# edlanglois/relearn

Hardware: AMD Instinct MI355X
Metric: env-steps/sec (whole node), 64k-env CartPole TRPO (higher is better)
Workload: dtype f32; 1 GPU; CartPole(VisibleStepLimit 500) MLP-TRPO, 65536 envs total, T=128, policy 5-128-2, critic 5-128-1, CG 10, <=15 backtracks, 80 Adam critic steps per period; n_envs_total=65536, n_envs_per_gpu=65536, horizon=128, hidden=128, critic_steps=80, update_chains=policy and critic chains side by side on two streams, pipeline=none, parallelism=env-sharded x1 + no collective (one rank)

## Files before the change

### include/relearn_hip.h

```cpp
#ifndef RELEARN_HIP_H
#define RELEARN_HIP_H

#include <stddef.h>
#include <stdint.h>

#ifdef __cplusplus
extern "C" {
#endif

#define RL_ABI_VERSION 6

typedef enum {
  RL_OK = 0,
  RL_ERR_INVALID_ARGUMENT = 1,
  RL_ERR_HIP = 2,
  RL_ERR_NO_DEVICE = 3,
  RL_ERR_BUILD_AGENT = 4,
  RL_ERR_BUILD_ENV = 5,
  RL_ERR_BUFFER_FULL = 6,
  RL_ERR_PACKING = 7,
  RL_ERR_COMM = 8,
  RL_ERR_OPT_NAN = 9,
  RL_ERR_UNSUPPORTED = 10
} rl_status;
// ... 82 lines not shown
int32_t rl_env_reset(rl_env *env);
int32_t rl_env_observe(rl_env *env, float *obs_out);
int32_t rl_env_step(rl_env *env, const uint8_t *actions, float *reward_out, uint8_t *flag_out, float *obs_out,
                    float *term_obs_out);
int32_t rl_env_upload_actions(rl_env *env, const uint8_t *actions);
int32_t rl_env_step_resident(rl_env *env);
int32_t rl_env_get_state(rl_env *env, double *state4, int32_t *nv_pos, uint64_t *steps_remaining,
                         uint64_t *reset_count);
int32_t rl_env_set_state(rl_env *env, const double *state4, const int32_t *nv_pos, const uint64_t *steps_remaining,
                         const uint64_t *reset_count);

int32_t rl_debug_stream_words(rl_engine *engine, uint64_t seed, uint64_t stream, uint64_t first_word, uint32_t n_words,
                              uint32_t *words_out);
int32_t rl_debug_device_memory(uint64_t *live_bytes, uint64_t *live_allocations);

int32_t rl_mlp_create(rl_engine *engine, uint32_t in_dim, uint32_t hidden, uint32_t out_dim, rl_mlp **out);
typedef enum {
  RL_ACT_IDENTITY = 0,
  RL_ACT_RELU = 1,
  RL_ACT_SIGMOID = 2,
  RL_ACT_TANH = 3
} rl_activation;
int32_t rl_mlp_create_layers(rl_engine *engine, uint32_t in_dim, const uint32_t *hidden_sizes, uint32_t n_hidden,
                             uint32_t out_dim, int32_t activation, int32_t output_activation, rl_mlp **out);
int32_t rl_mlp_create_config(rl_engine *engine, uint32_t in_dim, const uint32_t *hidden_sizes, uint32_t n_hidden,
                             uint32_t out_dim, int32_t activation, int32_t output_activation, int32_t bias, rl_mlp **out);
int32_t rl_mlp_destroy(rl_mlp *mlp);
int32_t rl_mlp_num_params(const rl_mlp *mlp, uint64_t *n);
int32_t rl_mlp_init(rl_mlp *mlp, uint64_t seed);
typedef enum { RL_INIT_ZEROS = 0, RL_INIT_CONSTANT = 1, RL_INIT_UNIFORM = 2, RL_INIT_NORMAL = 3, RL_INIT_ORTHOGONAL = 4 } rl_init_kind;
typedef enum { RL_SCALE_CONSTANT = 0, RL_SCALE_FAN_IN = 1, RL_SCALE_FAN_OUT = 2, RL_SCALE_FAN_AVG = 3 } rl_variance_scale;
typedef struct {
  int32_t kind;
  int32_t scale;
  double value;
} rl_initializer;
int32_t rl_mlp_init_with(rl_mlp *mlp, uint64_t seed, const rl_initializer *kernel_init, const rl_initializer *bias_init);
int32_t rl_rnn_mlp_init_with(rl_mlp *module, uint64_t seed, const rl_initializer *input_weights_init,
                             const rl_initializer *hidden_weights_init, const rl_initializer *bias_init,
                             const rl_initializer *mlp_kernel_init, const rl_initializer *mlp_bias_init);
int32_t rl_params_get(rl_mlp *mlp, float *host, uint64_t n);
int32_t rl_params_set(rl_mlp *mlp, const float *host, uint64_t n);
int32_t rl_mlp_forward(rl_mlp *mlp, const float *rows, uint64_t n_rows, float *out);

int32_t rl_gru_mlp_create(rl_engine *engine, uint32_t in_dim, uint32_t gru_hidden, uint32_t mlp_hidden,
                          uint32_t out_dim, rl_mlp **out);
int32_t rl_lstm_mlp_create(rl_engine *engine, uint32_t in_dim, uint32_t lstm_hidden, uint32_t mlp_hidden,
                           uint32_t out_dim, rl_mlp **out);
enum { RL_CELL_GRU = 0, RL_CELL_LSTM = 1 };
int32_t rl_rnn_mlp_create(rl_engine *engine, int32_t cell, uint32_t in_dim, uint32_t hidden_size, uint32_t num_layers,
                          uint32_t mlp_hidden, uint32_t out_dim, rl_mlp **out);
int32_t rl_rnn_mlp_create_config(rl_engine *engine, int32_t cell, uint32_t in_dim, uint32_t hidden_size,
                                 uint32_t num_layers, int32_t bias, uint32_t mlp_hidden, uint32_t out_dim, rl_mlp **out);

typedef enum {
  RL_TRAJ_OBS = 0,
  RL_TRAJ_ACTION = 1,
  RL_TRAJ_REWARD = 2,
  RL_TRAJ_FLAG = 3,
  RL_TRAJ_TERM_OBS = 4,
  RL_TRAJ_VALUES = 5,
  RL_TRAJ_ADVANTAGES = 6,
  RL_TRAJ_RETURNS = 7,
  RL_TRAJ_TARGETS = 8
} rl_traj_field;

int32_t rl_traj_create(rl_engine *engine, uint64_t n_lanes, uint64_t horizon, uint32_t obs_dim, rl_traj **out);
int32_t rl_traj_destroy(rl_traj *traj);
int32_t rl_traj_field_bytes(const rl_traj *traj, int32_t field, uint64_t *bytes);
int32_t rl_traj_read(rl_traj *traj, int32_t field, void *host, uint64_t bytes);
int32_t rl_traj_write(rl_traj *traj, int32_t field, const void *host, uint64_t bytes);

int32_t rl_rollout(rl_env *env, const rl_mlp *policy, rl_traj *traj);

int32_t rl_gae(rl_traj *traj, const rl_mlp *critic, float gamma, float lambda);
int32_t rl_seq_forward(rl_mlp *module, rl_traj *traj, float *out, float *succ_out);

typedef struct {
  uint64_t iterations;
  uint64_t max_backtracks;
  double backtrack_ratio;
  double hpv_reg_coeff;
  double max_policy_step_kl;
  int32_t accept_violation;
} rl_trpo_config;
int32_t rl_trpo_config_default(rl_trpo_config *cfg);

typedef struct {
  double entropy, step_size, loss_initial, loss_final, constraint_val_final, step_scale;
  int64_t num_backtracks;
  int32_t status;
  int32_t cg_iterations;
} rl_trpo_stats;

int32_t rl_trpo_update(rl_mlp *policy, rl_traj *traj, const rl_trpo_config *cfg, rl_trpo_stats *stats);
int32_t rl_policy_gradient(rl_mlp *policy, rl_traj *traj, float *grad_out, float *loss_out, float *entropy_out);
int32_t rl_policy_fvp(rl_mlp *policy, rl_traj *traj, const float *v, float reg, float *out);
int32_t rl_policy_loss_kl(rl_mlp *policy, rl_traj *traj, const float *params0, float *loss_out, float *kl_out);

typedef struct {
  double learning_rate, beta1, beta2, weight_decay;
  double eps;
} rl_adam_config;
int32_t rl_adam_config_default(rl_adam_config *cfg);
int32_t rl_adam_create(rl_mlp *module, const rl_adam_config *cfg, rl_adam **out);
int32_t rl_adam_destroy(rl_adam *opt);
int32_t rl_adam_step_host(rl_adam *opt, const float *grad);

enum { RL_OPTIMIZER_ADAM = 0, RL_OPTIMIZER_ADAMW = 1, RL_OPTIMIZER_SGD = 2, RL_OPTIMIZER_RMSPROP = 3 };
typedef struct {
  int32_t kind;
  int32_t nesterov;
  int32_t centered;
  int32_t reserved;
  double learning_rate, weight_decay;
  double beta1, beta2;
  double eps;
  double momentum, dampening;
  double alpha;
} rl_optimizer_config;
int32_t rl_optimizer_config_default(int32_t kind, rl_optimizer_config *cfg);
int32_t rl_optimizer_create(rl_mlp *module, const rl_optimizer_config *cfg, rl_adam **out);
int32_t rl_optimizer_step_host(rl_adam *opt, const float *grad);
int32_t rl_optimizer_state_read(rl_adam *opt, int32_t slot, float *host, uint64_t n, uint64_t *step_out);

typedef struct {
  double loss_first, loss_last;
  uint64_t steps;
} rl_critic_stats;
int32_t rl_critic_update(rl_mlp *critic, rl_adam *opt, rl_traj *traj, uint64_t opt_steps, rl_critic_stats *stats,
                         float *losses_out);
int32_t rl_critic_gradient(rl_mlp *critic, rl_traj *traj, float *grad_out, float *loss_out);

enum { RL_VALUE_TARGET_REWARD_TO_GO = 0, RL_VALUE_TARGET_ONE_STEP_TD = 1 };
typedef struct {
  uint64_t opt_steps_per_update;
  int32_t target;
  float discount_factor;
} rl_values_opt_config;
int32_t rl_values_opt_config_default(rl_values_opt_config *cfg);
int32_t rl_values_opt_update(rl_mlp *critic, rl_adam *opt, rl_traj *traj, const rl_values_opt_config *cfg,
                             rl_critic_stats *stats, float *losses_out );

int32_t rl_actor_critic_update(rl_mlp *policy, rl_mlp *critic, rl_adam *critic_opt, rl_traj *traj,
                               const rl_trpo_config *policy_cfg, const rl_values_opt_config *critic_cfg,
                               rl_trpo_stats *policy_stats, rl_critic_stats *critic_stats ,
                               float *critic_losses_out );
int32_t rl_actor_critic_update_begin(rl_mlp *policy, rl_mlp *critic, rl_adam *critic_opt, rl_traj *traj,
                                     const rl_trpo_config *policy_cfg, const rl_values_opt_config *critic_cfg,
                                     rl_trpo_stats *policy_stats);
int32_t rl_actor_critic_update_finish(rl_traj *traj, rl_critic_stats *critic_stats ,
                                      float *critic_losses_out );
int32_t rl_engine_set_serial_update(rl_engine *engine, int32_t serial);

typedef struct {
  uint64_t opt_steps_per_update;
  double clip_distance;
} rl_ppo_config;
int32_t rl_ppo_config_default(rl_ppo_config *cfg);
typedef struct {
  double entropy;
  double loss_first, loss_last;
  uint64_t steps;
} rl_policy_opt_stats;
int32_t rl_ppo_update(rl_mlp *policy, rl_adam *opt, rl_traj *traj, const rl_ppo_config *cfg,
                      rl_policy_opt_stats *stats, float *losses_out );
int32_t rl_reinforce_update(rl_mlp *policy, rl_adam *opt, rl_traj *traj, rl_policy_opt_stats *stats);
int32_t rl_reward_to_go(rl_traj *traj, float gamma);

enum { RL_DQN_TARGET_REWARD_TO_GO = 0, RL_DQN_TARGET_ONE_STEP_TD = 1 };
enum { RL_SCHEDULE_CONSTANT = 0, RL_SCHEDULE_LINEAR_ANNEALED = 1 };
enum { RL_COLLECT_CONSTANT = 0, RL_COLLECT_FIRST_REST = 1 };
typedef struct {
  int32_t target;
  int32_t exploration_kind;
  double exploration_start, exploration_end;
  uint64_t exploration_period;
  uint64_t minibatch_steps;
  uint64_t opt_steps_per_update;
  uint64_t buffer_capacity;
  uint64_t episode_capacity;
  int32_t update_kind;
  uint64_t update_first, update_rest;
  float discount_factor;
  uint32_t agent_key[8];
} rl_dqn_config;
int32_t rl_dqn_config_default(rl_dqn_config *cfg);
int32_t rl_dqn_create(rl_env *env, rl_mlp *qnet, rl_adam *opt, const rl_dqn_config *cfg, rl_dqn **out);
int32_t rl_dqn_destroy(rl_dqn *dqn);
int32_t rl_dqn_exploration_rate(const rl_dqn *dqn, int32_t training, double *rate_out);
int32_t rl_dqn_min_update_size(const rl_dqn *dqn, uint64_t *min_steps_out, uint64_t *slack_steps_out);
typedef struct {
  double exploration_rate;
  uint64_t steps;
  uint64_t episodes_ended;
} rl_dqn_collect_stats;
int32_t rl_dqn_collect(rl_dqn *dqn, uint64_t horizon, rl_dqn_collect_stats *stats );
typedef struct {
  double loss_first, loss_last;
  uint64_t opt_steps;
  uint64_t global_steps;
  uint64_t last_minibatch_steps, last_minibatch_episodes;
} rl_dqn_update_stats;
int32_t rl_dqn_update(rl_dqn *dqn, rl_dqn_update_stats *stats, float *losses_out );

enum { RL_REPLAY_HEAD = 0, RL_REPLAY_COUNT = 1, RL_REPLAY_EP_HEAD = 2, RL_REPLAY_EP_COUNT = 3, RL_REPLAY_TOTAL = 4,
       RL_REPLAY_EP_END = 5 , RL_REPLAY_OBS = 6 , RL_REPLAY_NEXT_OBS = 7,
       RL_REPLAY_ACTION = 8 , RL_REPLAY_REWARD = 9 , RL_REPLAY_FLAG = 10 ,
       RL_REPLAY_ACTOR_POS = 11 , RL_REPLAY_LAST_FLAGS = 12  };
int32_t rl_dqn_replay_field_bytes(const rl_dqn *dqn, int32_t field, uint64_t *bytes);
int32_t rl_dqn_replay_read(rl_dqn *dqn, int32_t field, void *host, uint64_t bytes);
int32_t rl_dqn_minibatch_sample(rl_dqn *dqn, int32_t sequential, uint64_t *n_episodes_out, uint64_t *n_steps_out);
enum { RL_MB_EP_LANE = 0, RL_MB_EP_START = 1, RL_MB_EP_LEN = 2, RL_MB_EP_OFFSET = 3 ,
       RL_MB_OBS = 4 , RL_MB_ACTION = 5 , RL_MB_TARGET = 6  };
int32_t rl_dqn_minibatch_read(rl_dqn *dqn, int32_t field, void *host, uint64_t bytes);
int32_t rl_dqn_minibatch_gradient(rl_dqn *dqn, float *grad_out, float *loss_out);
int32_t rl_dqn_agent_rng_pos(rl_dqn *dqn, uint64_t *pos_out);

typedef struct {
  double mean;
  double squared_residual_sum;
  uint64_t count;
} rl_mean_variance;
typedef struct {
  rl_mean_variance step_reward;
  rl_mean_variance episode_reward;
  rl_mean_variance episode_length;
} rl_steps_summary;
int32_t rl_summary_create(rl_engine *engine, uint64_t n_lanes, rl_summary **out);
int32_t rl_summary_destroy(rl_summary *s);
int32_t rl_summary_push(rl_summary *s, const rl_traj *traj);
int32_t rl_summary_push_dqn(rl_summary *s, const rl_dqn *dqn);
int32_t rl_summary_read(rl_summary *s, rl_steps_summary *out);
int32_t rl_summary_clear(rl_summary *s, int32_t forget_episodes_in_progress);
int32_t rl_steps_summary_merge(const rl_steps_summary *a, const rl_steps_summary *b, rl_steps_summary *out);

enum { RL_ACTOR_POLICY = 0, RL_ACTOR_DQN = 1 };
int32_t rl_actor_to_cbor(rl_env *env, rl_mlp *module, int32_t actor_kind, double exploration_rate, uint8_t *buf,
                         uint64_t cap, uint64_t *len_out);
int32_t rl_module_from_cbor(rl_mlp *module, const uint8_t *buf, uint64_t len);

typedef enum {
  RL_KIND_UINT8 = 0, RL_KIND_INT8 = 1, RL_KIND_INT16 = 2, RL_KIND_INT = 3, RL_KIND_INT64 = 4, RL_KIND_HALF = 5,
  RL_KIND_FLOAT = 6, RL_KIND_DOUBLE = 7, RL_KIND_COMPLEX_HALF = 8, RL_KIND_COMPLEX_FLOAT = 9,
  RL_KIND_COMPLEX_DOUBLE = 10, RL_KIND_BOOL = 11, RL_KIND_QINT8 = 12, RL_KIND_QUINT8 = 13, RL_KIND_QINT32 = 14,
  RL_KIND_BFLOAT16 = 15
} rl_tensor_kind;
int32_t rl_tensor_def_to_cbor(int32_t kind, const int64_t *shape, uint32_t rank, int32_t requires_grad,
                              const void *data, uint64_t data_bytes, uint8_t *buf, uint64_t cap, uint64_t *len_out);
int32_t rl_tensor_def_from_cbor(const uint8_t *buf, uint64_t len, int32_t *kind_out, int64_t *shape_out,
                                uint32_t shape_cap, uint32_t *rank_out, int32_t *requires_grad_out, void *data_out,
                                uint64_t data_cap, uint64_t *data_bytes_out);
int32_t rl_indexed_type_space_to_cbor(uint8_t *buf, uint64_t cap, uint64_t *len_out);

int32_t rl_chain_tabular_q_train(uint64_t seed, uint64_t n_threads, uint64_t n_periods, uint64_t min_worker_steps,
                                 double exploration_rate, double *q_values_out, uint64_t *counts_out,
                                 uint64_t *total_steps_out);
int32_t rl_chain_tabular_q_eval(const double *q_values, uint64_t seed, uint64_t n_steps, uint8_t *actions_out,
                                double *total_reward_out);

#ifdef __cplusplus
}
#endif
#endif
```

### relearn_amd/__init__.py

```python
import atexit
import ctypes as C
import math
import os
import subprocess
import sys
import weakref

import numpy as np

_HERE = os.path.dirname(os.path.abspath(__file__))
LIB_PATH = os.environ.get("RELEARN_LIB", os.path.join(_HERE, "librelearn_hip.so"))
CSRC = os.path.join(_HERE, "csrc")

OK = 0
ERR_INVALID_ARGUMENT, ERR_HIP, ERR_NO_DEVICE, ERR_BUILD_AGENT, ERR_BUILD_ENV = 1, 2, 3, 4, 5
ERR_BUFFER_FULL, ERR_PACKING, ERR_COMM, ERR_OPT_NAN, ERR_UNSUPPORTED = 6, 7, 8, 9, 10
SUCC_CONTINUE, SUCC_TERMINATE, SUCC_INTERRUPT = 0, 1, 2
OPT_OK, OPT_LOSS_NOT_IMPROVING, OPT_CONSTRAINT_VIOLATED, OPT_NAN_LOSS, OPT_NAN_CONSTRAINT = range(5)
ENV_CARTPOLE, ENV_CHAIN, ENV_MEMORY, ENV_BANDIT, ENV_META_BANDIT = 0, 1, 2, 3, 4
BANDITS_UNIFORM_BERNOULLI, BANDITS_ONE_HOT, BANDITS_ROUND_ROBIN = 0, 1, 2
BANDIT_DISTRIBUTIONS = {"uniform_bernoulli": BANDITS_UNIFORM_BERNOULLI, "one_hot": BANDITS_ONE_HOT,
                        "round_robin": BANDITS_ROUND_ROBIN}
LIMIT_NONE, LIMIT_LATENT, LIMIT_VISIBLE = 0, 1, 2
(TRAJ_OBS, TRAJ_ACTION, TRAJ_REWARD, TRAJ_FLAG, TRAJ_TERM_OBS, TRAJ_VALUES, TRAJ_ADVANTAGES,
 TRAJ_RETURNS, TRAJ_TARGETS) = range(9)
VALUE_TARGET_REWARD_TO_GO, VALUE_TARGET_ONE_STEP_TD = 0, 1
OPTIMIZER_ADAM, OPTIMIZER_ADAMW, OPTIMIZER_SGD, OPTIMIZER_RMSPROP = 0, 1, 2, 3
KERNEL_CLASSES = ["env_step", "rollout", "values", "gae", "policy_pass", "backward", "reduce", "small",
                  "critic_fwd", "allreduce", "critic_fused", "policy_fused", "policy_fvp"]

ABI_SYMBOLS = [
    "rl_abi_version", "rl_debug_stream_words", "rl_debug_device_memory", "rl_device_count", "rl_engine_create", "rl_engine_destroy", "rl_engine_sync",
    "rl_last_error", "rl_engine_info", "rl_engine_set_kernel_variant", "rl_timer_begin", "rl_timer_end", "rl_profile_enable", "rl_profile_read",
    "rl_comm_available", "rl_comm_library_paths", "rl_comm_unique_id", "rl_comm_init", "rl_comm_destroy", "rl_comm_init_host",
    "rl_comm_ipc_handle", "rl_comm_init_ipc", "rl_comm_selftest",
    "rl_cartpole_params_default", "rl_env_create", "rl_env_create_bandit", "rl_meta_bandit_config_default", "rl_env_create_meta_bandit", "rl_env_destroy", "rl_env_dims", "rl_env_reset",
    "rl_env_observe", "rl_env_step", "rl_env_upload_actions", "rl_env_step_resident", "rl_env_get_state",
    "rl_env_set_state",
    "rl_mlp_create", "rl_mlp_create_layers", "rl_mlp_create_config", "rl_mlp_destroy", "rl_mlp_num_params", "rl_mlp_init", "rl_mlp_init_with", "rl_params_get", "rl_params_set",
    "rl_mlp_forward", "rl_gru_mlp_create", "rl_lstm_mlp_create", "rl_rnn_mlp_create", "rl_rnn_mlp_create_config", "rl_rnn_mlp_init_with", "rl_seq_forward",
    "rl_traj_create", "rl_traj_destroy", "rl_traj_field_bytes", "rl_traj_read", "rl_traj_write",
    "rl_rollout", "rl_gae",
    "rl_trpo_config_default", "rl_trpo_update", "rl_policy_gradient", "rl_policy_fvp", "rl_policy_loss_kl",
    "rl_adam_config_default", "rl_adam_create", "rl_adam_destroy", "rl_adam_step_host",
    "rl_optimizer_config_default", "rl_optimizer_create", "rl_optimizer_step_host", "rl_optimizer_state_read",
    "rl_critic_update", "rl_critic_gradient", "rl_values_opt_config_default", "rl_values_opt_update",
    "rl_actor_critic_update", "rl_actor_critic_update_begin", "rl_actor_critic_update_finish", "rl_engine_set_serial_update",
    "rl_ppo_config_default", "rl_ppo_update", "rl_reinforce_update", "rl_reward_to_go",
    "rl_actor_to_cbor", "rl_module_from_cbor", "rl_tensor_def_to_cbor", "rl_tensor_def_from_cbor",
    "rl_indexed_type_space_to_cbor",
    "rl_dqn_config_default", "rl_dqn_create", "rl_dqn_destroy", "rl_dqn_exploration_rate",
    "rl_dqn_min_update_size", "rl_dqn_collect", "rl_dqn_update", "rl_dqn_replay_field_bytes", "rl_dqn_replay_read",
    "rl_dqn_minibatch_sample", "rl_dqn_minibatch_read", "rl_dqn_minibatch_gradient", "rl_dqn_agent_rng_pos",
    "rl_chain_tabular_q_train", "rl_chain_tabular_q_eval",
    "rl_summary_create", "rl_summary_destroy", "rl_summary_push", "rl_summary_push_dqn", "rl_summary_read",
    "rl_summary_clear", "rl_steps_summary_merge",
]


HOST_ALLREDUCE_FN = C.CFUNCTYPE(C.c_int32, C.c_void_p, C.POINTER(C.c_float), C.c_uint64)


class RelearnError(RuntimeError):
    def __init__(self, code, message):
        super().__init__("rl status %d: %s" % (code, message))
        self.code = code


class CartPoleParams(C.Structure):
    _fields_ = [(n, C.c_double) for n in (
        "gravity", "mass_cart", "mass_pole", "length_half_pole", "friction_cart", "friction_pole", "time_step",
        "action_force", "max_pos", "max_angle", "discount_factor")]


class EnvConfig(C.Structure):
    _fields_ = [("kind", C.c_int32), ("limit_kind", C.c_int32), ("max_steps", C.c_uint64), ("n_lanes", C.c_uint64),
                ("lane_offset", C.c_uint64), ("seed_env", C.c_uint64), ("seed_actor", C.c_uint64),
                ("cartpole", CartPoleParams), ("chain_size", C.c_uint64), ("memory_num_actions", C.c_uint64),
                ("memory_history_len", C.c_uint64), ("bandit_values", C.c_double * 2)]


class MetaBanditConfig(C.Structure):
    _fields_ = [("n_arms", C.c_uint32), ("distribution", C.c_int32), ("episodes_per_trial", C.c_uint64)]


class TrpoConfig(C.Structure):
    _fields_ = [("iterations", C.c_uint64), ("max_backtracks", C.c_uint64), ("backtrack_ratio", C.c_double),
                ("hpv_reg_coeff", C.c_double), ("max_policy_step_kl", C.c_double), ("accept_violation", C.c_int32)]


class TrpoStats(C.Structure):
    _fields_ = [("entropy", C.c_double), ("step_size", C.c_double), ("loss_initial", C.c_double),
                ("loss_final", C.c_double), ("constraint_val_final", C.c_double), ("step_scale", C.c_double),
                ("num_backtracks", C.c_int64), ("status", C.c_int32), ("cg_iterations", C.c_int32)]

    def as_dict(self):
        return {k: getattr(self, k) for k, _ in self._fields_}


class AdamConfig(C.Structure):
    _fields_ = [("learning_rate", C.c_double), ("beta1", C.c_double), ("beta2", C.c_double),
                ("weight_decay", C.c_double), ("eps", C.c_double)]


class OptimizerConfig(C.Structure):
    _fields_ = [("kind", C.c_int32), ("nesterov", C.c_int32), ("centered", C.c_int32), ("reserved", C.c_int32),
                ("learning_rate", C.c_double), ("weight_decay", C.c_double), ("beta1", C.c_double),
                ("beta2", C.c_double), ("eps", C.c_double), ("momentum", C.c_double), ("dampening", C.c_double),
                ("alpha", C.c_double)]


class CriticStats(C.Structure):
    _fields_ = [("loss_first", C.c_double), ("loss_last", C.c_double), ("steps", C.c_uint64)]


def build(force=False, check=False):
    if force or check or not os.path.exists(LIB_PATH):
        before = os.path.getmtime(LIB_PATH) if os.path.exists(LIB_PATH) else None
        subprocess.check_call(["make", "-C", CSRC, "-s", "-j4"] + (["-B"] if force else []))
        _write_build_record(before)
    return LIB_PATH


BUILD_RECORD = os.path.join(_HERE, "build_record.json")


def _write_build_record(mtime_before):
    import hashlib
    import json
    import time
    try:
        after = os.path.getmtime(LIB_PATH)
        try:
            hipcc = subprocess.run(["/opt/rocm/bin/hipcc", "--version"], capture_output=True, timeout=30).stdout.decode().splitlines()[0]
        except Exception:
            hipcc = None
        rec = {"mode": "linked a new library" if mtime_before is None or after > mtime_before else
                       "make: library newer than every source (nothing compiled)",
               "lib_sha16": hashlib.sha256(open(LIB_PATH, "rb").read()).hexdigest()[:16],
               "lib_mtime": time.strftime("%Y-%m-%dT%H:%M:%SZ", time.gmtime(after)),
               "checked_at": time.strftime("%Y-%m-%dT%H:%M:%SZ", time.gmtime()), "hipcc": hipcc,
               "arch": "gfx950"}
        json.dump(rec, open(BUILD_RECORD, "w"), indent=1)
    except Exception:
        pass


_lib = None


def lib():
    global _lib
    if _lib is None:
        if not os.path.exists(LIB_PATH):
            raise ImportError("librelearn_hip.so is not built: run `python -c 'import __graft_entry__ as g; "
                              "g.build()'` (there is no CPU fallback)")
        L = C.CDLL(LIB_PATH)
        L.rl_last_error.restype = C.c_char_p
        L.rl_last_error.argtypes = [C.c_void_p]
        _lib = L
    return _lib


def debug_device_memory():
    nbytes, count = C.c_uint64(), C.c_uint64()
    _check(lib().rl_debug_device_memory(C.byref(nbytes), C.byref(count)))
    return nbytes.value, count.value


def _check(code, eng=None):
    if code != OK:
        msg = lib().rl_last_error(eng)
        raise RelearnError(code, msg.decode() if msg else "")


def _ptr(a, dtype):
    a = np.ascontiguousarray(a, dtype=dtype)
    return a, a.ctypes.data_as(C.c_void_p)


_live = weakref.WeakSet()


def _register(obj):
    _live.add(obj)


@atexit.register
def _close_all():
    objs = list(_live)
    order = {"StepsSummary": -1, "Dqn": -1, "Adam": 0, "Optimizer": 0, "Trajectory": 1, "CartPoleEnv": 2, "ChainEnv": 2, "MetaBanditEnv": 2, "Mlp": 3, "GruMlp": 3,
             "Engine": 4}
    for o in sorted(objs, key=lambda o: order.get(type(o).__name__, 2)):
        o.close()


class _Handle:
    def __del__(self):
        if sys.is_finalizing():
            return
        try:
            self.close()
        except Exception:
            pass


class Engine(_Handle):
    def __init__(self, device=0):
        self.h = C.c_void_p()
        _check(lib().rl_engine_create(C.c_int32(device), C.byref(self.h)))
        _register(self)

    def close(self):
        if self.h:
            lib().rl_engine_destroy(self.h)
            self.h = C.c_void_p()

    def sync(self):
        _check(lib().rl_engine_sync(self.h), self.h)

    def info(self):
        name = C.create_string_buffer(256)
        arch = C.create_string_buffer(256)
        cus = C.c_int32()
        _check(lib().rl_engine_info(self.h, name, C.c_size_t(256), arch, C.c_size_t(256), C.byref(cus)), self.h)
        return name.value.decode(), arch.value.decode(), cus.value

    def stream_words(self, seed, stream, first_word, n_words):
        out = np.zeros(n_words, dtype=np.uint32)
        _check(lib().rl_debug_stream_words(self.h, C.c_uint64(seed), C.c_uint64(stream), C.c_uint64(first_word),
                                           C.c_uint32(n_words), out.ctypes.data_as(C.c_void_p)), self.h)
        return out

    def set_kernel_variant(self, variant):
        _check(lib().rl_engine_set_kernel_variant(self.h, C.c_int32(variant)), self.h)

    def set_serial_update(self, serial):
        _check(lib().rl_engine_set_serial_update(self.h, C.c_int32(1 if serial else 0)), self.h)

    def timer_begin(self):
        _check(lib().rl_timer_begin(self.h), self.h)

    def timer_end(self):
        ms = C.c_float()
        _check(lib().rl_timer_end(self.h, C.byref(ms)), self.h)
        return ms.value

    def profile_enable(self, on=True):
        _check(lib().rl_profile_enable(self.h, C.c_int32(1 if on else 0)), self.h)

    def profile_read(self, reset=True):
        ms = (C.c_double * len(KERNEL_CLASSES))()
        cnt = (C.c_uint64 * len(KERNEL_CLASSES))()
        _check(lib().rl_profile_read(self.h, ms, cnt, C.c_int32(1 if reset else 0)), self.h)
        return {k: (ms[i], cnt[i]) for i, k in enumerate(KERNEL_CLASSES)}

    def comm_init(self, rank, n_ranks, unique_id):
        buf = (C.c_uint8 * 128).from_buffer_copy(bytes(unique_id))
        _check(lib().rl_comm_init(self.h, C.c_int32(rank), C.c_int32(n_ranks), buf), self.h)

    def comm_ipc_handle(self, n_ranks):
        buf = (C.c_uint8 * 64)()
        _check(lib().rl_comm_ipc_handle(self.h, C.c_int32(n_ranks), buf), self.h)
        return bytes(buf)

    def comm_init_ipc(self, rank, n_ranks, handles):
        blob = b"".join(bytes(h) for h in handles)
        assert len(blob) == 64 * n_ranks
        buf = (C.c_uint8 * len(blob)).from_buffer_copy(blob)
        _check(lib().rl_comm_init_ipc(self.h, C.c_int32(rank), C.c_int32(n_ranks), buf), self.h)

    def comm_selftest(self):
        _check(lib().rl_comm_selftest(self.h), self.h)

    def comm_destroy(self):
        _check(lib().rl_comm_destroy(self.h), self.h)
        self._host_allreduce = None

    def comm_init_host(self, rank, n_ranks, allreduce):
        def thunk(_ctx, buf, count):
            try:
                allreduce(np.ctypeslib.as_array(buf, shape=(count,)))
                return 0
            except Exception:
                import traceback
                traceback.print_exc()
                return 1
        self._host_allreduce = HOST_ALLREDUCE_FN(thunk)
        _check(lib().rl_comm_init_host(self.h, C.c_int32(rank), C.c_int32(n_ranks), self._host_allreduce, None),
               self.h)


def comm_available():
    return lib().rl_comm_available() == OK


def comm_library_paths():
    a, b = C.create_string_buffer(1024), C.create_string_buffer(1024)
    _check(lib().rl_comm_library_paths(a, C.c_size_t(1024), b, C.c_size_t(1024)))
    return a.value.decode(), b.value.decode()


def comm_unique_id():
    buf = (C.c_uint8 * 128)()
    _check(lib().rl_comm_unique_id(buf))
    return bytes(buf)


def cartpole_params_default():
    p = CartPoleParams()
    _check(lib().rl_cartpole_params_default(C.byref(p)))
    return p


class CartPoleEnv(_Handle):

    def __init__(self, engine, n_lanes, max_steps=500, limit=LIMIT_VISIBLE, lane_offset=0, seed_env=0,
                 seed_actor=1, params=None):
        self.eng = engine
        cfg = EnvConfig()
        cfg.kind = ENV_CARTPOLE
        cfg.limit_kind = limit
        cfg.max_steps = max_steps
        cfg.n_lanes = n_lanes
        cfg.lane_offset = lane_offset
        cfg.seed_env = seed_env
        cfg.seed_actor = seed_actor
        cfg.cartpole = params if params is not None else cartpole_params_default()
        self.cfg = cfg
        self.h = C.c_void_p()
        _check(lib().rl_env_create(engine.h, C.byref(cfg), C.byref(self.h)), engine.h)
        _register(self)
        self.n = n_lanes
        d, a = C.c_uint32(), C.c_uint32()
        _check(lib().rl_env_dims(self.h, C.byref(d), C.byref(a)), engine.h)
        self.D, self.A = d.value, a.value

    def close(self):
        if self.h:
            lib().rl_env_destroy(self.h)
            self.h = C.c_void_p()

    def reset(self):
        _check(lib().rl_env_reset(self.h), self.eng.h)

    def observe(self):
        obs = np.zeros((self.D, self.n), dtype=np.float32)
        _check(lib().rl_env_observe(self.h, obs.ctypes.data_as(C.c_void_p)), self.eng.h)
        return obs

    def step(self, actions):
        a, ap = _ptr(actions, np.uint8)
        assert a.shape == (self.n,)
        reward = np.zeros(self.n, dtype=np.float32)
        flag = np.zeros(self.n, dtype=np.uint8)
        obs = np.zeros((self.D, self.n), dtype=np.float32)
        term = np.zeros((self.D, self.n), dtype=np.float32)
        _check(lib().rl_env_step(self.h, ap, reward.ctypes.data_as(C.c_void_p), flag.ctypes.data_as(C.c_void_p),
                                 obs.ctypes.data_as(C.c_void_p), term.ctypes.data_as(C.c_void_p)), self.eng.h)
        return reward, flag, obs, term

    def upload_actions(self, actions):
        a, ap = _ptr(actions, np.uint8)
        _check(lib().rl_env_upload_actions(self.h, ap), self.eng.h)

    def step_resident(self):
        _check(lib().rl_env_step_resident(self.h), self.eng.h)

    def get_state(self):
        st = np.zeros((4, self.n), dtype=np.float64)
        nv = np.zeros(self.n, dtype=np.int32)
        rem = np.zeros(self.n, dtype=np.uint64)
        rc = np.zeros(self.n, dtype=np.uint64)
        _check(lib().rl_env_get_state(self.h, st.ctypes.data_as(C.c_void_p), nv.ctypes.data_as(C.c_void_p),
                                      rem.ctypes.data_as(C.c_void_p), rc.ctypes.data_as(C.c_void_p)), self.eng.h)
        return st, nv, rem, rc

    def set_state(self, st, nv, rem, rc):
        st, sp = _ptr(st, np.float64)
        nv, np_ = _ptr(nv, np.int32)
        rem, rp = _ptr(rem, np.uint64)
        rc, cp = _ptr(rc, np.uint64)
        _check(lib().rl_env_set_state(self.h, sp, np_, rp, cp), self.eng.h)


class ChainEnv(_Handle):

    def __init__(self, engine, n_lanes, max_steps=100, limit=LIMIT_LATENT, lane_offset=0, seed_env=0, seed_actor=1):
        self.eng = engine
        cfg = EnvConfig()
        cfg.kind = ENV_CHAIN
        cfg.limit_kind = limit
# ... 746 lines not shown
```

### relearn_amd/csrc/abi.hip

```cpp
#include <dlfcn.h>

#include <atomic>
#include <condition_variable>
#include <map>
#include <mutex>

#include "abi_internal.hpp"
#include "env_lanes.hpp"

thread_local std::string g_last_error_no_engine;

static std::atomic<uint64_t> g_device_bytes{0}, g_device_allocations{0};

void *rl_device_alloc(uint64_t bytes) {
  void *p = nullptr;
  RL_HIP_CHECK(hipMalloc(&p, bytes));
  g_device_bytes += bytes;
  g_device_allocations += 1;
  return p;
}

void rl_device_free(void *p, uint64_t bytes) {
  (void)hipFree(p);
  g_device_bytes -= bytes;
// ... 170 lines not shown
    RL_HIP_CHECK(hipStreamSynchronize(e->stream));
    return;
  }
  if (!e->comm) {
    if (e->n_ranks > 1) throw RlError(RL_ERR_COMM, "engine has n_ranks > 1 but no collective (rl_comm_init failed?)");
    return;
  }
  ProfScope ps(e, RL_K_ALLREDUCE);
  void *comm = e->chan == 1 && e->comm_aux ? e->comm_aux : e->comm;
  rccl_check(g_rccl.AllReduce(d_buf, d_buf, count, 7, 0, comm, e->stream), "ncclAllReduce");
}

void comm_agree(rl_engine *e) {
  const bool mine = std::getenv("RELEARN_SERIAL_UPDATE") != nullptr;
  if (!e->has_collective()) {
    e->agreed_serial_env = mine;
    return;
  }
  float h[2] = {mine ? 1.0f : 0.0f, 1.0f};
  {
    DevMem tmp;
    float *d = tmp.alloc<float>(2);
    h2d(e, d, h, sizeof(h));
    rl_allreduce_sum_f32(e, d, 2);
    d2h(e, h, d, sizeof(h));
    ipc_check(e);
  }
  if (h[1] != (float)e->n_ranks)
    throw RlError(RL_ERR_COMM, "the collective's first all-reduce counted " + std::to_string((int)h[1]) + " of " +
                                   std::to_string(e->n_ranks) + " ranks");
  e->agreed_serial_env = h[0] != 0.0f;
}

extern "C" {

int32_t rl_abi_version(void) { return RL_ABI_VERSION; }

int32_t rl_device_count(int32_t *count) {
  return guarded(nullptr, [&] {
    RL_REQUIRE(count, "count is NULL");
    int n = 0;
    if (hipGetDeviceCount(&n) != hipSuccess) n = 0;
    *count = n;
  });
}

int32_t rl_engine_create(int32_t device_ordinal, rl_engine **out) {
  return guarded(nullptr, [&] {
    RL_REQUIRE(out, "out is NULL");
    *out = nullptr;
    int n = 0;
    if (hipGetDeviceCount(&n) != hipSuccess || n <= 0)
      throw RlError(RL_ERR_NO_DEVICE, "no HIP device visible: this engine has no CPU fallback");
    RL_REQUIRE(device_ordinal >= 0 && device_ordinal < n, "device ordinal out of range");
    std::unique_ptr<rl_engine> e(new rl_engine());
    e->device = device_ordinal;
    RL_HIP_CHECK(hipSetDevice(device_ordinal));
    RL_HIP_CHECK(hipGetDeviceProperties(&e->prop, device_ordinal));
    if (std::strncmp(e->prop.gcnArchName, "gfx950", 6) != 0)
      throw RlError(RL_ERR_NO_DEVICE,
                    std::string("device is ") + e->prop.gcnArchName + ", this library is built for gfx950 only");
    RL_HIP_CHECK(hipStreamCreateWithFlags(&e->main_stream, hipStreamNonBlocking));
    RL_HIP_CHECK(hipStreamCreateWithFlags(&e->aux_stream, hipStreamNonBlocking));
    e->stream = e->main_stream;
    RL_HIP_CHECK(hipEventCreateWithFlags(&e->ev_fork, hipEventDisableTiming));
    RL_HIP_CHECK(hipEventCreateWithFlags(&e->ev_join, hipEventDisableTiming));
    RL_HIP_CHECK(hipEventCreate(&e->ev_begin));
    RL_HIP_CHECK(hipEventCreate(&e->ev_end));
    e->pinned_bytes = 1 << 16;
    RL_HIP_CHECK(hipHostMalloc(&e->pinned, e->pinned_bytes, hipHostMallocDefault));
    *out = e.release();
  });
}

static void engine_teardown(rl_engine *e);

int32_t rl_engine_destroy(rl_engine *e) {
  if (!e) return RL_OK;
  if (e->live_handles > 0) {
    e->zombie = true;
    return RL_OK;
  }
  engine_teardown(e);
  return RL_OK;
}

void engine_release_child(rl_engine *e) {
  e->live_handles -= 1;
  if (e->zombie && e->live_handles <= 0) engine_teardown(e);
}

static void engine_teardown(rl_engine *e) {
  (void)hipSetDevice(e->device);
  (void)hipStreamSynchronize(e->main_stream);
  (void)hipStreamSynchronize(e->aux_stream);
  if (e->comm_aux && g_rccl.CommDestroy) g_rccl.CommDestroy(e->comm_aux);
  if (e->comm && g_rccl.CommDestroy) g_rccl.CommDestroy(e->comm);
  ipc_teardown(e);
  prof_drain(e);
  for (auto ev : e->prof_event_pool) (void)hipEventDestroy(ev);
  if (e->pinned) (void)hipHostFree(e->pinned);
  (void)hipEventDestroy(e->ev_begin);
  (void)hipEventDestroy(e->ev_end);
  (void)hipEventDestroy(e->ev_fork);
  (void)hipEventDestroy(e->ev_join);
  (void)hipStreamDestroy(e->aux_stream);
  (void)hipStreamDestroy(e->main_stream);
  delete e;
}

int32_t rl_engine_sync(rl_engine *e) {
  return guarded(e, [&] {
    RL_REQUIRE(e, "engine is NULL");
    sync(e);
    RL_HIP_CHECK(hipSetDevice(e->device));
    RL_HIP_CHECK(hipDeviceSynchronize());
    ipc_check(e);
  });
}

const char *rl_last_error(const rl_engine *e) { return e ? e->last_error.c_str() : g_last_error_no_engine.c_str(); }

int32_t rl_engine_info(const rl_engine *e, char *name_out, size_t name_cap, char *arch_out, size_t arch_cap,
                       int32_t *compute_units) {
  return guarded(const_cast<rl_engine *>(e), [&] {
    RL_REQUIRE(e, "engine is NULL");
    if (name_out && name_cap) std::snprintf(name_out, name_cap, "%s", e->prop.name[0] ? e->prop.name : e->prop.gcnArchName);
    if (arch_out && arch_cap) std::snprintf(arch_out, arch_cap, "%s", e->prop.gcnArchName);
    if (compute_units) *compute_units = e->prop.multiProcessorCount;
  });
}

int32_t rl_timer_begin(rl_engine *e) {
  return guarded(e, [&] {
    RL_REQUIRE(e, "engine is NULL");
    RL_HIP_CHECK(hipEventRecord(e->ev_begin, e->stream));
  });
}

int32_t rl_timer_end(rl_engine *e, float *elapsed_ms) {
  return guarded(e, [&] {
    RL_REQUIRE(e && elapsed_ms, "NULL argument");
    RL_HIP_CHECK(hipEventRecord(e->ev_end, e->stream));
    RL_HIP_CHECK(hipEventSynchronize(e->ev_end));
    RL_HIP_CHECK(hipEventElapsedTime(elapsed_ms, e->ev_begin, e->ev_end));
  });
}

int32_t rl_engine_set_kernel_variant(rl_engine *e, int32_t variant) {
  return guarded(e, [&] {
    RL_REQUIRE(e, "engine is NULL");
    RL_REQUIRE(variant == 0 || variant == 1, "kernel variant must be 0 (best) or 1 (v1 reference kernels)");
    e->kernel_variant = variant;
  });
}

int32_t rl_engine_set_serial_update(rl_engine *e, int32_t serial) {
  return guarded(e, [&] {
    RL_REQUIRE(e, "engine is NULL");
    e->serial_update = serial != 0;
  });
}

int32_t rl_profile_enable(rl_engine *e, int32_t on) {
  return guarded(e, [&] {
    RL_REQUIRE(e, "engine is NULL");
    sync(e);
    prof_drain(e);
    e->profiling = on != 0;
  });
}

int32_t rl_profile_read(rl_engine *e, double *total_ms_out, uint64_t *launches_out, int32_t reset) {
  return guarded(e, [&] {
    RL_REQUIRE(e, "engine is NULL");
    sync(e);
    prof_drain(e);
    for (int i = 0; i < RL_K_CLASS_COUNT; ++i) {
      if (total_ms_out) total_ms_out[i] = e->prof_ms[i];
      if (launches_out) launches_out[i] = e->prof_launches[i];
      if (reset) {
        e->prof_ms[i] = 0.0;
        e->prof_launches[i] = 0;
      }
    }
  });
}

int32_t rl_comm_available(void) {
  return guarded(nullptr, [&] {
    if (std::getenv("RELEARN_LOOPBACK_COMM")) return;
    rccl_load();
  });
}

int32_t rl_comm_library_paths(char *rccl_out, size_t rccl_cap, char *hip_out, size_t hip_cap) {
  return guarded(nullptr, [&] {
    Dl_info info;
    if (rccl_out && rccl_cap) {
      rccl_out[0] = 0;
      if (g_rccl.AllReduce && dladdr((void *)g_rccl.AllReduce, &info) != 0 && info.dli_fname)
        std::snprintf(rccl_out, rccl_cap, "%s", info.dli_fname);
    }
    if (hip_out && hip_cap) {
      hip_out[0] = 0;
      if (dladdr((void *)&hipGetDeviceCount, &info) != 0 && info.dli_fname)
        std::snprintf(hip_out, hip_cap, "%s", info.dli_fname);
    }
  });
}

int32_t rl_comm_unique_id(uint8_t id_out[128]) {
  return guarded(nullptr, [&] {
    RL_REQUIRE(id_out, "id_out is NULL");
    if (std::getenv("RELEARN_LOOPBACK_COMM")) {
      static std::atomic<uint64_t> counter{0};
      std::memset(id_out, 0, 128);
      uint64_t v = ++counter;
      std::memcpy(id_out, &v, sizeof(v));
      return;
    }
    rccl_load();
    rccl_check(g_rccl.GetUniqueId(id_out), "ncclGetUniqueId");
  });
}

int32_t rl_comm_init(rl_engine *e, int32_t rank, int32_t n_ranks, const uint8_t unique_id[128]) {
  return guarded(e, [&] {
    RL_REQUIRE(e && unique_id, "NULL argument");
    RL_REQUIRE(n_ranks >= 1 && rank >= 0 && rank < n_ranks, "bad rank / n_ranks");
    RL_REQUIRE(!e->has_collective(), "communicator already initialised");
    if (std::getenv("RELEARN_LOOPBACK_COMM")) {
      RL_REQUIRE(!e->loopback, "communicator already initialised");
      std::lock_guard<std::mutex> lk(g_loopback_mu);
      std::string key((const char *)unique_id, 128);
      auto &grp = g_loopback_groups[key];
      if (!grp) {
        grp = std::make_shared<LoopbackGroup>();
        grp->n_ranks = n_ranks;
        grp->bufs.assign(n_ranks, nullptr);
        RL_HIP_CHECK(hipSetDevice(e->device));
        RL_HIP_CHECK(hipMalloc((void **)&grp->d_bufs, n_ranks * sizeof(float *)));
        if (const char *tw = std::getenv("RELEARN_LOOPBACK_TEST_WEIGHT")) {
          int r = -1;
          float w = 1.0f;
          if (std::sscanf(tw, "%d:%f", &r, &w) == 2 && r >= 0 && r < n_ranks) grp->bad_rank = r, grp->bad_weight = w;
        }
      }
      RL_REQUIRE(grp->n_ranks == n_ranks, "loopback group: inconsistent n_ranks");
      grp->joined += 1;
      e->loopback = grp.get();
      e->rank = rank;
      e->n_ranks = n_ranks;
      e->agreed_serial_env = std::getenv("RELEARN_SERIAL_UPDATE") != nullptr;
      return;
    }
    if (n_ranks == 1 && !std::getenv("RELEARN_FORCE_RCCL")) return;
    rccl_load();
    RL_HIP_CHECK(hipSetDevice(e->device));
    UniqueId id;
    std::memcpy(id.bytes, unique_id, 128);
    comm_init_rank_t init = (comm_init_rank_t)(void *)g_rccl.CommInitRank;
    void *comm = nullptr;
    rccl_check(init(&comm, n_ranks, id, rank), "ncclCommInitRank");
    e->comm = comm;
    e->rank = rank;
    e->n_ranks = n_ranks;
    try {
      const bool want_aux = std::getenv("RELEARN_NO_AUX_COMM") == nullptr;
      UniqueId id2;
      std::memset(id2.bytes, 0, sizeof(id2.bytes));
      bool id_ok = false;
      if (rank == 0 && want_aux) id_ok = g_rccl.GetUniqueId(id2.bytes) == 0;
      float h_id[130];
      for (int i = 0; i < 128; ++i) h_id[i] = rank == 0 && id_ok ? (float)(unsigned char)id2.bytes[i] : 0.0f;
      h_id[128] = rank == 0 && !id_ok ? 1.0f : 0.0f;
      h_id[129] = want_aux ? 0.0f : 1.0f;
      DevMem tmp;
      float *d_id = tmp.alloc<float>(130);
      void *comm2 = nullptr;
      try {
        h2d(e, d_id, h_id, sizeof(h_id));
        rccl_check(g_rccl.AllReduce(d_id, d_id, 130, 7, 0, e->comm, e->stream), "ncclAllReduce (second unique id)");
        d2h(e, h_id, d_id, sizeof(h_id));
        const bool attempt = h_id[128] == 0.0f && h_id[129] == 0.0f;
        float outcome = 0.0f;
        if (attempt) {
          for (int i = 0; i < 128; ++i) id2.bytes[i] = (char)(unsigned char)h_id[i];
          if (init(&comm2, n_ranks, id2, rank) == 0 && comm2 != nullptr) outcome = 1.0f;
          else comm2 = nullptr;
        }
        h2d(e, d_id, &outcome, sizeof(outcome));
        rccl_check(g_rccl.AllReduce(d_id, d_id, 1, 7, 0, e->comm, e->stream), "ncclAllReduce (second communicator: outcome)");
        d2h(e, &outcome, d_id, sizeof(outcome));
        if (outcome == (float)n_ranks) {
          e->comm_aux = comm2;
          comm2 = nullptr;
        } else {
          if (rank == 0)
            std::fprintf(stderr, "relearn_hip: no second communicator (%s): update chains will run one after the other "
                                 "on every rank\n",
                         !attempt ? (h_id[129] != 0.0f ? "RELEARN_NO_AUX_COMM on some rank" : "rank 0 could not make an id")
                                  : "ncclCommInitRank failed on some rank");
        }
      } catch (...) {
        if (comm2) g_rccl.CommDestroy(comm2);
// ... 1101 lines not shown
```

### relearn_amd/csrc/abi_internal.hpp

```cpp
#pragma once
#include <cmath>
#include <cstdlib>
#include <cstring>
#include <memory>
#include <string>
#include <vector>

#include "../../include/rl_chacha.h"
#include "../../include/rl_detmath.h"
#include "engine.hpp"
#include "host/cbor.hpp"
#include "kernels.hpp"

extern thread_local std::string g_last_error_no_engine;

static inline void engine_settle(rl_engine *e) {
  if (e->pending.active && !e->pending.joined) {
    RL_HIP_CHECK(hipStreamWaitEvent(e->main_stream, e->ev_join, 0));
    e->pending.joined = true;
  }
}

template <typename F>
static inline int32_t guarded(rl_engine *eng, F &&f, bool settle = true) {
  try {
    if (eng != nullptr) eng->call_epoch += 1;
    if (eng != nullptr && settle) engine_settle(eng);
    f();
    if (eng != nullptr) {
      const hipError_t le = hipGetLastError();
      if (le != hipSuccess) throw RlError(RL_ERR_HIP, std::string("kernel launch failed: ") + hipGetErrorString(le));
    }
    return RL_OK;
  } catch (const RlError &e) {
    if (eng != nullptr) eng->error_epoch += 1;
    (eng ? eng->last_error : g_last_error_no_engine) = e.what();
    return e.code;
  } catch (const std::exception &e) {
    if (eng != nullptr) eng->error_epoch += 1;
    (eng ? eng->last_error : g_last_error_no_engine) = e.what();
    return RL_ERR_INVALID_ARGUMENT;
  } catch (...) {
    if (eng != nullptr) eng->error_epoch += 1;
    (eng ? eng->last_error : g_last_error_no_engine) = "unknown error";
    return RL_ERR_INVALID_ARGUMENT;
  }
}

static inline uint64_t b_total(const rl_traj *t) { return t->B * (uint64_t)t->eng->n_ranks; }

static inline void sync(rl_engine *e) { RL_HIP_CHECK(hipStreamSynchronize(e->stream)); }

static inline void h2d(rl_engine *e, void *d, const void *h, size_t bytes) {
  RL_HIP_CHECK(hipMemcpyAsync(d, h, bytes, hipMemcpyHostToDevice, e->stream));
  sync(e);
}

static inline void d2h(rl_engine *e, void *h, const void *d, size_t bytes) {
  RL_HIP_CHECK(hipMemcpyAsync(h, d, bytes, hipMemcpyDeviceToHost, e->stream));
  sync(e);
}

constexpr uint32_t RL_GUARD_BOTH = (1u << RL_GUARD_POLICY) | (1u << RL_GUARD_CRITIC);
static inline void range_check(rl_traj *t, uint32_t chains = RL_GUARD_BOTH) {
  if (chains & (1u << RL_GUARD_POLICY)) t->guard_next_policy = true;
  if (chains & (1u << RL_GUARD_CRITIC)) t->guard_next_critic = true;
  if (t->h_range_err == nullptr) return;
  volatile uint32_t *w = t->h_range_err;
  uint32_t seen = 0u;
  for (int c = 0; c < 2; ++c)
    if ((chains & (1u << c)) != 0u && w[c] != 0u) seen |= 1u << c;
  if (seen == 0u) return;
  for (int c = 0; c < 2; ++c)
    if (seen & (1u << c)) {
      w[c] = 0u;
      RL_HIP_CHECK(hipMemsetAsync(t->d.range + RL_RANGE_WORDS + c, 0, sizeof(uint32_t), t->eng->stream));
    }
  sync(t->eng);
  throw RlError(RL_ERR_UNSUPPORTED,
                std::string("numeric range of the fused update kernels exceeded in the ") +
                    (seen == RL_GUARD_BOTH ? "policy and critic chains" : (seen & 1u) ? "policy chain" : "critic chain") +
                    " (|pre-activation| bound 2^31 or a non-zero pre-activation below 2^-46 possible, or a non-finite "
                    "observation): the result of this call is not valid and the update was not applied; use "
                    "rl_engine_set_kernel_variant(engine, 1) for these magnitudes (include/relearn_hip.h)");
}
static inline void range_discard(rl_traj *t) {
  try {
    range_check(t);
  } catch (const RlError &) {
  }
}

enum PassKind { RUN_INIT = PASS_INIT, RUN_EVAL = PASS_EVAL, RUN_JVP = PASS_JVP, RUN_DQN = PASS_DQN, RUN_PPO = PASS_PPO,
                RUN_CRITIC, RUN_KINDS };
struct SlabRows {
  uint32_t A, B;
};
struct PassRequest {
  PassRequest(PassKind k) : kind(k) {}
  PassKind kind;
  const float *tangent = nullptr;
  const int32_t *skip = nullptr;
  float clip_lo = 0.0f, clip_hi = 0.0f;
  bool forward_only = false;
  bool reduce = true;
  uint64_t B_total = 0;
};
SlabRows run_pass(const rl_mlp *mod, rl_traj *traj, const PassRequest &req);

extern "C" {
void engine_release_child(rl_engine *e);
void traj_plan(rl_traj *t, uint64_t B);
rl_traj *traj_alloc(rl_engine *e, uint64_t n_lanes, uint64_t horizon, uint32_t obs_dim, bool resizable);
void seq_ensure(rl_traj *t, const rl_mlp *mod, bool training);
void traj_ensure_pvec(rl_traj *t, uint64_t P);
rl_mlp *seq_exec(const rl_mlp *m);
}

struct SeqScope {
  rl_traj *t;
  uint32_t logical_D;
  rl_mlp *x;
  SeqScope(rl_traj *traj, const rl_mlp *m) : t(traj), logical_D(traj->d.D), x(nullptr) {
    RL_REQUIRE(m->in_dim == traj->d.D, "module input width does not match the trajectory");
    x = seq_exec(m);
    if (!m->lane_kernels()) t->d.D = 5;
  }
  ~SeqScope() { t->d.D = logical_D; }
  SeqScope(const SeqScope &) = delete;
  SeqScope &operator=(const SeqScope &) = delete;
};
```

### relearn_amd/csrc/abi_update.hip

```cpp
#include "abi_internal.hpp"

enum FusedLauncher { FUSED_NONE, FUSED_POLICY ,
                     FUSED_CRITIC  };
struct PassRow {
  bool backward, sums;
  FusedLauncher fused;
};
static const PassRow PASS_TABLE[RUN_KINDS] = {
     {true, true, FUSED_POLICY},
     {false, true, FUSED_POLICY},
     {true, false, FUSED_POLICY},
     {true, true, FUSED_NONE},
     {true, true, FUSED_POLICY},
     {true, true, FUSED_CRITIC},
};
static_assert(RUN_INIT == 0 && RUN_EVAL == 1 && RUN_JVP == 2 && RUN_DQN == 3 && RUN_PPO == 4 && RUN_CRITIC == 5 &&
                  RUN_KINDS == 6,
              "PASS_TABLE rows are in the order of PassKind");

static void seq_gradient_to_flat_order(const rl_mlp *mod, rl_traj *traj) {
  if (mod->exec == nullptr) return;
  launch_seq_unpad(mod, traj->vec, mod->x_tmp);
  RL_HIP_CHECK(hipMemcpyAsync(traj->vec, mod->x_tmp, mod->P * sizeof(float), hipMemcpyDeviceToDevice, traj->eng->stream));
}

static float *seq_record(rl_traj *traj, const rl_mlp *mod) {
  return mod->lane_kernels() ? traj->seq.stack.rec : traj->seq.act;
}

SlabRows run_pass(const rl_mlp *mod, rl_traj *traj, const PassRequest &req) {
  const PassRow &row = PASS_TABLE[req.kind];
  const bool critic = req.kind == RUN_CRITIC;
  const uint32_t P = (uint32_t)mod->P;
  const uint64_t Bt = req.B_total ? req.B_total : b_total(traj);
  bool grad = row.backward;
  auto allreduce = [&] {
    rl_allreduce_sum_f32(traj->eng, traj->vec + (grad ? 0 : P), (grad ? P : 0) + (row.sums ? 4 : 0));
  };
  if (rl_module_is_recurrent(mod->kind)) {
    RL_REQUIRE(req.reduce, "a recurrent pass reduces its own sums");
    grad = row.backward && !req.forward_only;
    SeqScope sc(traj, mod);
    seq_ensure(traj, sc.x, true);
    if (req.kind == RUN_JVP) {
      const float *tangent = req.tangent;
      if (mod->exec != nullptr) {
        launch_seq_pad(mod, mod->x_tan, req.tangent);
        tangent = mod->x_tan;
      }
      launch_gru_tangent(traj, sc.x, tangent, Bt, req.skip);
    } else {
      launch_gru_seq_forward(traj, sc.x, traj->seq.out, nullptr, grad ? seq_record(traj, sc.x) : nullptr, req.skip);
      if (critic) launch_seq_critic_dvalues(traj, Bt);
      else launch_seq_policy_dlogits(traj, req.kind, Bt, req.clip_lo, req.clip_hi, req.skip);
    }
    if (grad) {
      launch_gru_backward(traj, sc.x, req.skip);
      seq_gradient_to_flat_order(mod, traj);
    }
    if (row.sums) launch_reduce(traj, P, false, true, 0, traj->nbB);
    allreduce();
    return SlabRows{0, traj->nbB};
  }
  bool fused = false;
  if (traj->eng->kernel_variant == 0) {
    if (row.fused == FUSED_POLICY)
      fused = launch_policy_v2(traj, mod, req.kind, req.tangent, Bt, req.skip, req.clip_lo, req.clip_hi);
    else if (row.fused == FUSED_CRITIC)
      fused = launch_critic_step_v2(traj, mod, Bt);
  }
  if (!fused) {
    if (critic) launch_critic_fwd(traj, mod, Bt);
    else launch_policy_pass(traj, mod, req.kind, req.tangent, Bt, req.skip, req.clip_lo, req.clip_hi);
    if (row.backward) launch_mlp_backward(traj, mod, req.skip);
  }
  const SlabRows rows = fused ? SlabRows{traj->last_rows, traj->last_rows} : SlabRows{traj->nbA, traj->nbB};
  if (req.reduce) {
    launch_reduce(traj, P, row.backward, row.sums, rows.A, rows.B);
    allreduce();
  }
  return rows;
}

extern "C" {

int32_t rl_trpo_config_default(rl_trpo_config *c) {
  return guarded(nullptr, [&] {
    RL_REQUIRE(c, "cfg is NULL");
    c->iterations = 10;
    c->max_backtracks = 15;
    c->backtrack_ratio = 0.8;
    c->hpv_reg_coeff = 1e-5;
    c->max_policy_step_kl = 0.01;
    c->accept_violation = 0;
  });
}

static void check_policy(const rl_mlp *policy, const rl_traj *traj) {
  RL_REQUIRE(policy && traj, "NULL argument");
  RL_REQUIRE(policy->eng == traj->eng, "handles belong to different engines");
  RL_REQUIRE(policy->in_dim == traj->d.D && policy->out_dim >= 2, "policy shape does not match the trajectory");
  RL_REQUIRE(traj->n_actions == 0 || policy->out_dim == traj->n_actions,
             "policy outputs do not match the action count of the env this trajectory was collected on");
  RL_REQUIRE(policy->out_dim > traj->max_action, "the trajectory holds an action index the policy has no output for");
  if (policy->out_dim > 2 && policy->kind != RL_MODULE_MLP)
    throw RlError(RL_ERR_UNSUPPORTED, "recurrent chains are built for two actions");
}

static inline void trpo_candidate(rl_mlp *policy, rl_traj *traj, const rl_trpo_config *cfg, uint64_t i, double ratio) {
  launch_ls_set_params(traj, policy, ratio);
  PassRequest eval(RUN_EVAL);
  eval.skip = &traj->trpo->ls_accepted;
  run_pass(policy, traj, eval);
  launch_ls_check(traj, (uint32_t)policy->P, b_total(traj), (int)i, ratio, cfg->max_policy_step_kl);
}

struct TrpoProgress {
  uint64_t next = 0;
  double ratio = 1.0;
};

static TrpoProgress trpo_update_head(rl_mlp *policy, rl_traj *traj, const rl_trpo_config *cfg) {
  uint32_t P = (uint32_t)policy->P;
  uint64_t Bt = b_total(traj);
  float reg = (float)cfg->hpv_reg_coeff;
  run_pass(policy, traj, RUN_INIT);
  launch_trpo_begin(traj, policy, Bt);
  PassRequest fvp(RUN_JVP);
  fvp.tangent = traj->cg_p;
  fvp.skip = &traj->trpo->cg_done;
  for (uint64_t it = 0; it < cfg->iterations; ++it) {
    run_pass(policy, traj, fvp);
    launch_cg_step(traj, P, reg, 1e-10f);
  }
  launch_cg_finish(traj, P);
  fvp.tangent = traj->cg_x;
  fvp.skip = nullptr;
  run_pass(policy, traj, fvp);
  launch_step_size(traj, policy, reg, cfg->max_policy_step_kl);
  TrpoProgress pr;
  for (; pr.next < cfg->max_backtracks && pr.next < 2; ++pr.next) {
    if (pr.next > 0) pr.ratio *= cfg->backtrack_ratio;
    trpo_candidate(policy, traj, cfg, pr.next, pr.ratio);
  }
  return pr;
}

static void trpo_update_tail(rl_mlp *policy, rl_traj *traj, const rl_trpo_config *cfg, TrpoProgress pr,
                             rl_trpo_stats *stats) {
  rl_engine *e = traj->eng;
  double ratio = pr.ratio;
  for (uint64_t i = pr.next; i < cfg->max_backtracks; ++i) {
    if ((i & 1) == 0) {
      int32_t accepted = 0;
      d2h(e, &accepted, &traj->trpo->ls_accepted, sizeof(accepted));
      if (accepted != 0) break;
    }
    ratio *= cfg->backtrack_ratio;
    trpo_candidate(policy, traj, cfg, i, ratio);
  }
  launch_ls_finalize(traj, policy, cfg->max_policy_step_kl, cfg->accept_violation);
  TrpoStateDev h;
  d2h(e, &h, traj->trpo, sizeof(h));
  ipc_check(e);
  range_check(traj, 1u << RL_GUARD_POLICY);
  stats->entropy = (double)h.entropy;
  stats->step_size = h.step_size;
  stats->loss_initial = (double)h.loss0;
  stats->loss_final = (double)h.ls_loss;
  stats->constraint_val_final = (double)h.ls_kl;
  stats->step_scale = h.ls_accepted ? h.ls_ratio : 0.0;
  stats->num_backtracks = h.ls_accepted ? (int64_t)h.ls_index : -1;
  stats->status = h.status;
  stats->cg_iterations = h.cg_iters;
}

static void trpo_update_impl(rl_mlp *policy, rl_traj *traj, const rl_trpo_config *cfg, rl_trpo_stats *stats) {
  trpo_update_tail(policy, traj, cfg, trpo_update_head(policy, traj, cfg), stats);
}

static void trpo_raise_nan(const rl_trpo_stats *stats) {
  if (stats->status == RL_OPT_NAN_LOSS || stats->status == RL_OPT_NAN_CONSTRAINT)
    throw RlError(RL_ERR_OPT_NAN, stats->status == RL_OPT_NAN_LOSS ? "NaN loss in policy optimization"
                                                                   : "NaN constraint in policy optimization");
}

int32_t rl_trpo_update(rl_mlp *policy, rl_traj *traj, const rl_trpo_config *cfg, rl_trpo_stats *stats) {
  return guarded(traj ? traj->eng : nullptr, [&] {
    check_policy(policy, traj);
    RL_REQUIRE(cfg && stats, "NULL argument");
    trpo_update_impl(policy, traj, cfg, stats);
    trpo_raise_nan(stats);
  });
}

int32_t rl_policy_gradient(rl_mlp *policy, rl_traj *traj, float *grad_out, float *loss_out, float *entropy_out) {
  return guarded(traj ? traj->eng : nullptr, [&] {
    check_policy(policy, traj);
    RL_REQUIRE(grad_out, "grad_out is NULL");
    uint32_t P = (uint32_t)policy->P;
    run_pass(policy, traj, RUN_INIT);
    std::vector<float> h(P + 4);
    d2h(traj->eng, h.data(), traj->vec, (P + 4) * sizeof(float));
    range_check(traj, 1u << RL_GUARD_POLICY);
    std::memcpy(grad_out, h.data(), P * sizeof(float));
    double inv_B = 1.0 / (double)b_total(traj);
    if (loss_out) *loss_out = (float)(-((double)h[P] * inv_B));
    if (entropy_out) *entropy_out = (float)((double)h[P + 1] * inv_B);
  });
}

int32_t rl_policy_fvp(rl_mlp *policy, rl_traj *traj, const float *v, float reg, float *out) {
  return guarded(traj ? traj->eng : nullptr, [&] {
    check_policy(policy, traj);
    RL_REQUIRE(v && out, "NULL argument");
    uint32_t P = (uint32_t)policy->P;
    run_pass(policy, traj, RUN_INIT);
    h2d(traj->eng, traj->cg_x, v, P * sizeof(float));
    PassRequest fvp(RUN_JVP);
    fvp.tangent = traj->cg_x;
    run_pass(policy, traj, fvp);
    std::vector<float> h(P);
    d2h(traj->eng, h.data(), traj->vec, P * sizeof(float));
    range_check(traj, 1u << RL_GUARD_POLICY);
    for (uint32_t i = 0; i < P; ++i) out[i] = h[i] + reg * v[i];
  });
}

int32_t rl_policy_loss_kl(rl_mlp *policy, rl_traj *traj, const float *params0, float *loss_out, float *kl_out) {
  return guarded(traj ? traj->eng : nullptr, [&] {
    check_policy(policy, traj);
    RL_REQUIRE(params0 && loss_out && kl_out, "NULL argument");
    rl_engine *e = traj->eng;
    uint32_t P = (uint32_t)policy->P;
    uint64_t Bt = b_total(traj);
    std::vector<float> cur(P);
    d2h(e, cur.data(), policy->d_params, P * sizeof(float));
    h2d(e, policy->d_params, params0, P * sizeof(float));
    wimg_invalidate(policy);
    run_pass(policy, traj, RUN_INIT);
    h2d(e, policy->d_params, cur.data(), P * sizeof(float));
    wimg_invalidate(policy);
    run_pass(policy, traj, RUN_EVAL);
    float h[4];
    d2h(e, h, traj->vec + P, sizeof(h));
    range_check(traj, 1u << RL_GUARD_POLICY);
    double inv_B = 1.0 / (double)Bt;
    *loss_out = (float)(-((double)h[0] * inv_B));
    *kl_out = (float)((double)h[1] * inv_B);
  });
}

int32_t rl_adam_config_default(rl_adam_config *c) {
  return guarded(nullptr, [&] {
    RL_REQUIRE(c, "cfg is NULL");
    c->learning_rate = 1e-3;
    c->beta1 = 0.9;
    c->beta2 = 0.999;
    c->weight_decay = 0.0;
    c->eps = 1e-8;
  });
}

static void optimizer_config_default(int32_t kind, rl_optimizer_config *c) {
  std::memset(c, 0, sizeof(*c));
  c->kind = kind;
  c->eps = 1e-8;
  if (kind == RL_OPTIMIZER_ADAM || kind == RL_OPTIMIZER_ADAMW) {
    c->learning_rate = 1e-3;
    c->beta1 = 0.9;
    c->beta2 = 0.999;
  } else if (kind == RL_OPTIMIZER_SGD) {
    c->learning_rate = 1e-2;
  } else if (kind == RL_OPTIMIZER_RMSPROP) {
    c->learning_rate = 1e-2;
    c->alpha = 0.99;
  } else {
    throw RlError(RL_ERR_INVALID_ARGUMENT, "optimizer config: unknown kind");
  }
}

int32_t rl_optimizer_config_default(int32_t kind, rl_optimizer_config *c) {
  return guarded(nullptr, [&] {
    RL_REQUIRE(c, "cfg is NULL");
    optimizer_config_default(kind, c);
  });
}

static void optimizer_config_check(const rl_optimizer_config &c) {
  const int32_t k = c.kind;
  RL_REQUIRE(k == RL_OPTIMIZER_ADAM || k == RL_OPTIMIZER_ADAMW || k == RL_OPTIMIZER_SGD || k == RL_OPTIMIZER_RMSPROP,
             "optimizer config: unknown kind");
  RL_REQUIRE(c.learning_rate >= 0.0, "optimizer config: invalid learning_rate (negative)");
  RL_REQUIRE(c.weight_decay >= 0.0, "optimizer config: invalid weight_decay (negative)");
  if (k == RL_OPTIMIZER_ADAM || k == RL_OPTIMIZER_ADAMW) {
    RL_REQUIRE(c.eps >= 0.0, "optimizer config: invalid eps (negative)");
    RL_REQUIRE(c.beta1 >= 0.0 && c.beta1 < 1.0, "optimizer config: invalid beta1 (outside [0, 1))");
    RL_REQUIRE(c.beta2 >= 0.0 && c.beta2 < 1.0, "optimizer config: invalid beta2 (outside [0, 1))");
  } else if (k == RL_OPTIMIZER_SGD) {
    RL_REQUIRE(c.momentum >= 0.0, "optimizer config: invalid momentum (negative)");
    RL_REQUIRE(!c.nesterov || (c.momentum > 0.0 && c.dampening == 0.0),
               "optimizer config: nesterov requires a momentum > 0 and zero dampening");
  } else {
    RL_REQUIRE(c.eps >= 0.0, "optimizer config: invalid eps (negative)");
    RL_REQUIRE(c.momentum >= 0.0, "optimizer config: invalid momentum (negative)");
    RL_REQUIRE(c.alpha >= 0.0, "optimizer config: invalid alpha (negative)");
  }
}

static bool optimizer_has_slot(const rl_optimizer_config &c, int slot) {
  if (c.kind == RL_OPTIMIZER_ADAM || c.kind == RL_OPTIMIZER_ADAMW) return slot < 2;
  if (c.kind == RL_OPTIMIZER_SGD) return slot == 0 && c.momentum != 0.0;
  return slot == 0 || (slot == 1 && c.momentum > 0.0) || (slot == 2 && c.centered != 0);
}

static void optimizer_create(rl_mlp *module, const rl_optimizer_config &cfg, rl_adam **out) {
  rl_engine *e = module->eng;
  RL_HIP_CHECK(hipSetDevice(e->device));
  std::unique_ptr<rl_adam> o(new rl_adam());
  o->eng = e;
  o->mod = module;
  o->cfg = cfg;
  o->error_epoch = e->error_epoch;
  for (int s = 0; s < 3; ++s)
    if (optimizer_has_slot(cfg, s)) {
      o->d_state[s] = o->mem.alloc<float>(module->P);
      RL_HIP_CHECK(hipMemsetAsync(o->d_state[s], 0, module->P * sizeof(float), e->stream));
    }
  o->d_step = o->mem.alloc<uint64_t>(1);
  RL_HIP_CHECK(hipMemsetAsync(o->d_step, 0, sizeof(uint64_t), e->stream));
  sync(e);
  e->live_handles += 1;
  *out = o.release();
}

int32_t rl_adam_create(rl_mlp *module, const rl_adam_config *cfg, rl_adam **out) {
  return guarded(module ? module->eng : nullptr, [&] {
    RL_REQUIRE(module && cfg && out, "NULL argument");
    *out = nullptr;
    rl_optimizer_config c;
    optimizer_config_default(RL_OPTIMIZER_ADAM, &c);
    c.learning_rate = cfg->learning_rate;
    c.beta1 = cfg->beta1;
    c.beta2 = cfg->beta2;
    c.weight_decay = cfg->weight_decay;
    c.eps = cfg->eps;
    optimizer_create(module, c, out);
  });
}

int32_t rl_optimizer_create(rl_mlp *module, const rl_optimizer_config *cfg, rl_adam **out) {
  return guarded(module ? module->eng : nullptr, [&] {
    RL_REQUIRE(cfg, "cfg is NULL");
    optimizer_config_check(*cfg);
    RL_REQUIRE(module && out, "NULL argument");
    *out = nullptr;
    optimizer_create(module, *cfg, out);
  });
}

int32_t rl_adam_destroy(rl_adam *o) {
  if (!o) return RL_OK;
  (void)hipSetDevice(o->eng->device);
  (void)hipStreamSynchronize(o->eng->stream);
  (void)hipStreamSynchronize(o->eng->aux_stream);
  rl_engine *eng = o->eng;
  delete o;
  engine_release_child(eng);
  return RL_OK;
}
// ... 388 lines not shown
```

### relearn_amd/csrc/bf16_tile.hpp

```cpp
#pragma once
#include <hip/hip_runtime.h>

#include <cstdint>
#include <type_traits>

#include "../../include/rl_detmath.h"

namespace bt {

typedef float f32x16 __attribute__((ext_vector_type(16)));
typedef float f32x2 __attribute__((ext_vector_type(2)));
typedef __bf16 bf16x8 __attribute__((ext_vector_type(8)));
typedef __bf16 bf16x2 __attribute__((ext_vector_type(2)));

constexpr int NT = 4;
constexpr int PAR_D = 5, PAR_H = 128;
constexpr uint32_t PAR_B1 = PAR_H * PAR_D, PAR_W2 = PAR_B1 + PAR_H;
__host__ __device__ constexpr uint32_t par_b2(int A) { return PAR_W2 + (uint32_t)(A * PAR_H); }
constexpr uint32_t SHARE_OLD = 5, SHARE_YOUNG = 3;

__device__ __forceinline__ void wave_lds_fence() {
  __builtin_amdgcn_fence(__ATOMIC_RELEASE, "wavefront");
  __builtin_amdgcn_wave_barrier();
  __builtin_amdgcn_fence(__ATOMIC_ACQUIRE, "wavefront");
// ... 86 lines not shown
  }
  uint32_t p0, p1, p2;
  split3(FWD_SCALE * w, p0, p1, p2);
  const unsigned short q0 = (unsigned short)p0, q1 = (unsigned short)p1, q2 = (unsigned short)p2;
  auto put = [&](int t, int lane, int h) {
    h16[wimg_half_index(t, lane, h)] = q0;
    h16[wimg_half_index(t, lane, h + 1)] = q1;
    h16[wimg_half_index(t, lane, h + 2)] = q2;
  };
  if (p >= PAR_B1) {
    const int j = (int)(p - PAR_B1), t = j >> 5, n = j & 31;
    put(t, 32 + n, 21);
    f32[wimg_raw_index(t, 32 + n, 2)] = w;
    return;
  }
  const int j = (int)p / D, k = (int)p % D, t = j >> 5, n = j & 31;
  if (k < 4) {
    const int lane = n + 32 * (k >> 1), base = 9 * (k & 1);
    put(t, lane, base);
    put(t, lane, base + 3);
    put(t, lane, base + 6);
    f32[wimg_raw_index(t, lane, k & 1)] = w;
  } else {
    put(t, n, 18);
    put(t, n, 21);
    put(t, 32 + n, 18);
    f32[wimg_raw_index(t, n, 2)] = w;
  }
}
struct WRaw {
  float wa, wb, wc, w2[2];
};
__device__ __forceinline__ void wimg_load(const uint32_t *__restrict__ img, int t, int lane, Frag (&f)[3], WRaw &r, int A);

__device__ __forceinline__ void input_frags(float xa, float xb, float xc, bool valid, int hf, Frag (&f)[3]) {
  uint32_t a0, a1, a2, c0, c1, c2, e0, e1, e2;
  split3t(xa, a0, a1, a2);
  split3t(xb, c0, c1, c2);
  split3t(xc, e0, e1, e2);
  const uint32_t one = valid ? 0x3F800000u : 0u;
  const uint32_t x0 = hf == 0 ? e0 : e2, x1 = hf == 0 ? e1 : one;
  f[0].u[0] = pkh(a0, a0);
  f[0].u[1] = pkh(a0, a1);
  f[0].u[2] = pkh(a1, a1);
  f[0].u[3] = pkh(a2, a2);
  f[1].u[0] = pkh(a2, c0);
  f[1].u[1] = pkh(c0, c0);
  f[1].u[2] = pkh(c1, c1);
  f[1].u[3] = pkh(c1, c2);
  f[2].u[0] = pkh(c2, c2);
  f[2].u[1] = pkh(x0, x0);
  f[2].u[2] = pkh(x0, x1);
  f[2].u[3] = pkh(x1, x1);
}

__device__ __forceinline__ void wimg_load(const uint32_t *__restrict__ img, int t, int lane, Frag (&f)[3], WRaw &r, int A) {
  const uint4 *__restrict__ fi = reinterpret_cast<const uint4 *>(img);
  const float *__restrict__ rw = reinterpret_cast<const float *>(img);
#pragma unroll
  for (int i = 0; i < 3; ++i) f[i].x = fi[(t * 3 + i) * 64 + lane];
  r.wa = rw[wimg_raw_index(t, lane, 0)];
  r.wb = rw[wimg_raw_index(t, lane, 1)];
  r.wc = rw[wimg_raw_index(t, lane, 2)];
  r.w2[0] = rw[wimg_raw_index(t, lane, 3)];
  r.w2[1] = A > 1 ? rw[wimg_raw_index(t, lane, 4)] : 0.0f;
}
__device__ __forceinline__ f32x16 layer1(const Frag (&fa)[3], const Frag (&fw)[3]) {
  f32x16 c = {0, 0, 0, 0, 0, 0, 0, 0, 0, 0, 0, 0, 0, 0, 0, 0};
#pragma unroll
  for (int i = 0; i < 3; ++i) c = __builtin_amdgcn_mfma_f32_32x32x16_bf16(fa[i].v, fw[i].v, c, 0, 0, 0);
  return c;
}


constexpr int RANGE_SLOTS = 64, RANGE_STRIDE = 32;
constexpr int RANGE_WORDS = 2 * RANGE_SLOTS * RANGE_STRIDE;
constexpr int GUARD_POLICY = 0, GUARD_CRITIC = 1;
constexpr int RANGE_ALLOC_WORDS = RANGE_WORDS + RANGE_STRIDE;
__device__ __forceinline__ uint32_t *range_veto(uint32_t *range, int chain) { return range + RANGE_WORDS + chain; }
__device__ __forceinline__ uint32_t *range_lo_slot(uint32_t *range, int s) { return range + s * RANGE_STRIDE; }
__device__ __forceinline__ uint32_t *range_hi_slot(uint32_t *range, int s) { return range + (RANGE_SLOTS + s) * RANGE_STRIDE; }
__device__ __forceinline__ void range_fold(uint32_t *range, uint32_t workgroup, uint32_t lo, uint32_t hi) {
  const int s = (int)(workgroup % RANGE_SLOTS);
  if (lo < __hip_atomic_load(range_lo_slot(range, s), __ATOMIC_RELAXED, __HIP_MEMORY_SCOPE_AGENT)) atomicMin(range_lo_slot(range, s), lo);
  if (hi > __hip_atomic_load(range_hi_slot(range, s), __ATOMIC_RELAXED, __HIP_MEMORY_SCOPE_AGENT)) atomicMax(range_hi_slot(range, s), hi);
}
__device__ __forceinline__ void range_reset(uint32_t *range, int tid, int nthreads) {
  for (int s = tid; s < RANGE_SLOTS; s += nthreads) {
    *range_lo_slot(range, s) = 0x7F7FFFFFu;
    *range_hi_slot(range, s) = 0u;
  }
}
__device__ __forceinline__ void range_accumulate(float x, uint32_t &lo, uint32_t &hi) {
  const uint32_t a = __builtin_bit_cast(uint32_t, x) & 0x7FFFFFFFu;
  hi = a > hi ? a : hi;
  lo = a != 0u && a < lo ? a : lo;
}
__device__ __forceinline__ void range_fold_wave(uint32_t *range, uint32_t key, uint32_t lo, uint32_t hi) {
#pragma unroll
  for (int m = 32; m > 0; m >>= 1) {
    const uint32_t ol = (uint32_t)__shfl_xor((int)lo, m, 64), oh = (uint32_t)__shfl_xor((int)hi, m, 64);
    lo = ol < lo ? ol : lo;
    hi = oh > hi ? oh : hi;
  }
  if ((threadIdx.x & 63) == 0) range_fold(range, key, lo, hi);
}
__device__ __forceinline__ void range_bounds(uint32_t *range, int lane, float &xmin, float &xmax) {
  uint32_t lo = *range_lo_slot(range, lane % RANGE_SLOTS), hi = *range_hi_slot(range, lane % RANGE_SLOTS);
#pragma unroll
  for (int m = 32; m > 0; m >>= 1) {
    const uint32_t ol = (uint32_t)__shfl_xor((int)lo, m, 64), oh = (uint32_t)__shfl_xor((int)hi, m, 64);
    lo = ol < lo ? ol : lo;
    hi = oh > hi ? oh : hi;
  }
  xmax = __builtin_bit_cast(float, hi);
  xmin = hi == 0u ? 0.0f : __builtin_bit_cast(float, lo);
}
__device__ __forceinline__ void range_guard(float wa, float wb, float w4, float bj, int hf, float xmin, float xmax,
                                            uint32_t *err, uint32_t *veto) {
  const float aa = __builtin_fabsf(wa), ab = __builtin_fabsf(wb);
  const float own = hf == 0 ? __builtin_fabsf(w4) : 0.0f, bias = __builtin_fabsf(bj);
  float hi = (aa + ab + own) * xmax, lo = __builtin_fmaxf(__builtin_fmaxf(aa, ab), own) * xmin, nz = aa + ab + own;
  float hi0, hi1, lo0, lo1, nz0, nz1;
  both_halves(hi, hi0, hi1);
  both_halves(lo, lo0, lo1);
  both_halves(nz, nz0, nz1);
  const float upper = hi0 + hi1 + bias, largest = __builtin_fmaxf(__builtin_fmaxf(lo0, lo1), bias);
  const bool zero_unit = nz0 + nz1 + bias == 0.0f;
  const bool bad = !(upper < 0x1p31f) || (!zero_unit && !(largest >= 0x1p-46f));
  if (bad) {
    __hip_atomic_store(veto, 1u, __ATOMIC_RELAXED, __HIP_MEMORY_SCOPE_AGENT);
    __hip_atomic_store(err, 1u, __ATOMIC_RELAXED, __HIP_MEMORY_SCOPE_SYSTEM);
  }
}
__device__ __forceinline__ void range_guard_img(const WRaw &r, int hf, float xmin, float xmax, uint32_t *err,
                                                uint32_t *veto) {
  float w4, bj;
  both_halves(r.wc, w4, bj);
  range_guard(r.wa, r.wb, w4, bj, hf, xmin, xmax, err, veto);
}

__device__ __forceinline__ uint32_t mask_pair(float lo, float hi, float after) {
  uint32_t r;
  asm("v_cvt_pk_bf16_f32 %0, %1, %2 clamp" : "=v"(r) : "v"(lo), "v"(hi), "v"(after));
  return r;
}
__device__ __forceinline__ void mask_tile(const f32x16 &c, Frag (&ga)[2]) {
  const float first = __builtin_amdgcn_fmed3f(c[0], 0.0f, 1.0f);
#pragma unroll
  for (int s = 0; s < 2; ++s)
#pragma unroll
    for (int i = 0; i < 4; ++i)
      ga[s].u[i] = mask_pair(s + i == 0 ? first : c[8 * s + 2 * i], c[8 * s + 2 * i + 1], first);
}

constexpr int L2_KS = 8;
__device__ __forceinline__ constexpr int acc_row(int s, int h, int e) { return 16 * s + 8 * (e >> 2) + 4 * h + (e & 3); }
__device__ __forceinline__ void ident_frags(int lane, Frag (&id)[2]) {
  const int n = lane & 31, hh = lane >> 5;
#pragma unroll
  for (int s = 0; s < 2; ++s)
#pragma unroll
    for (int i = 0; i < 4; ++i)
      id[s].u[i] = pk(acc_row(s, hh, 2 * i) == n ? 0x3F80u : 0u, acc_row(s, hh, 2 * i + 1) == n ? 0x3F80u : 0u);
}
template <typename F>
__device__ __forceinline__ void l2_build(uint4 (*img)[64], int tid, int nthreads, F val) {
  for (int idx = tid; idx < L2_KS * 64; idx += nthreads) {
    const int ks = idx >> 6, ln = idx & 63, m = ln & 31, hh = ln >> 5;
    const int hf_out = (m >> 2) & 1, r = (m & 3) + 4 * (m >> 3), i = r / 3, p = r % 3;
    const int k = i < 2 ? 2 * hf_out + i : 4 + hf_out;
    uint32_t h[8];
#pragma unroll
    for (int e = 0; e < 8; ++e) {
      uint32_t q0, q1, q2;
      split3(val(32 * (ks >> 1) + acc_row(ks & 1, hh, e), k), q0, q1, q2);
      h[e] = r < 9 ? (p == 0 ? q0 : (p == 1 ? q1 : q2)) : 0u;
    }
    img[ks][ln] = make_uint4(pk(h[0], h[1]), pk(h[2], h[3]), pk(h[4], h[5]), pk(h[6], h[7]));
  }
}
__device__ __forceinline__ f32x16 masked_sum_tile(const Frag (&ga)[2], const Frag (&idb)[2], const uint4 (*img)[64],
                                                  int t, int lane, f32x16 q) {
  f32x16 gt = {0, 0, 0, 0, 0, 0, 0, 0, 0, 0, 0, 0, 0, 0, 0, 0};
  gt = __builtin_amdgcn_mfma_f32_32x32x16_bf16(ga[0].v, idb[0].v, gt, 0, 0, 0);
  gt = __builtin_amdgcn_mfma_f32_32x32x16_bf16(ga[1].v, idb[1].v, gt, 0, 0, 0);
#pragma unroll
  for (int s = 0; s < 2; ++s) {
    Frag mt, fz;
#pragma unroll
    for (int i = 0; i < 4; ++i) mt.u[i] = pack_bf16(gt[8 * s + 2 * i], gt[8 * s + 2 * i + 1]);
    fz.x = img[2 * t + s][lane];
    q = __builtin_amdgcn_mfma_f32_32x32x16_bf16(fz.v, mt.v, q, 0, 0, 0);
  }
  return q;
}
__device__ __forceinline__ float l2_dot(const f32x16 &q, float xa, float xb, float xc) {
  const float sa = (q[0] + q[1]) + q[2], sb = (q[3] + q[4]) + q[5], sc = (q[6] + q[7]) + q[8];
  return __builtin_fmaf(xc, sc, __builtin_fmaf(xb, sb, xa * sa));
}

struct Pieces3 {
  uint32_t p[3];
};
__device__ __forceinline__ Pieces3 split3v(float v) {
  Pieces3 r;
  split3t(v, r.p[0], r.p[1], r.p[2]);
  return r;
}
__device__ __forceinline__ void piece_operand(const Pieces3 &a, const Pieces3 &b, const Pieces3 &c, Frag (&pa)[2]) {
  pa[0].u[0] = pkh(a.p[0], a.p[1]);
  pa[0].u[1] = pkh(a.p[2], b.p[0]);
  pa[0].u[2] = pkh(b.p[1], b.p[2]);
  pa[0].u[3] = pkh(c.p[0], c.p[1]);
  pa[1].u[0] = c.p[2] >> 16;
  pa[1].u[1] = pa[1].u[2] = pa[1].u[3] = 0u;
}
__device__ __forceinline__ void sel_frags(int lane, Frag (&sel)[2]) {
  const int n = lane & 31, hh = lane >> 5;
  auto col = [&](int i) {
    const int q = i / 3, p = i % 3;
    return (q == 0 ? 6 * hh : (q == 1 ? 6 * hh + 3 : (hh == 0 ? 12 : 16))) + p;
  };
#pragma unroll
  for (int i = 0; i < 4; ++i) sel[0].u[i] = pk(col(2 * i) == n ? 0x3F80u : 0u, col(2 * i + 1) == n ? 0x3F80u : 0u);
  sel[1].u[0] = col(8) == n ? 0x3F80u : 0u;
  sel[1].u[1] = sel[1].u[2] = sel[1].u[3] = 0u;
}
__device__ __forceinline__ void piece_frags_mfma(float g, float xa, float xb, float xc, int hf, const Frag (&sel)[2],
                                                 Frag (&ub)[2]) {
  Frag pa[2];
  piece_operand(split3v(g * xa), split3v(g * xb), split3v(hf == 0 ? g * xc : g), pa);
  f32x16 ut = {0, 0, 0, 0, 0, 0, 0, 0, 0, 0, 0, 0, 0, 0, 0, 0};
  ut = __builtin_amdgcn_mfma_f32_32x32x16_bf16(pa[0].v, sel[0].v, ut, 0, 0, 0);
  ut = __builtin_amdgcn_mfma_f32_32x32x16_bf16(pa[1].v, sel[1].v, ut, 0, 0, 0);
#pragma unroll
  for (int s = 0; s < 2; ++s)
#pragma unroll
    for (int i = 0; i < 4; ++i) ub[s].u[i] = pack_bf16(ut[8 * s + 2 * i], ut[8 * s + 2 * i + 1]);
}

__device__ __forceinline__ void backward(const Frag (&ga)[NT][2], const Frag (&ub)[2], f32x16 (&dm)[NT]) {
#pragma unroll
  for (int t = 0; t < NT; ++t)
#pragma unroll
    for (int s = 0; s < 2; ++s) dm[t] = __builtin_amdgcn_mfma_f32_32x32x16_bf16(ga[t][s].v, ub[s].v, dm[t], 0, 0, 0);
}

__device__ __forceinline__ void flush(f32x16 (&dm)[NT], double *acc64, int stride, int n, int hf, bool first = false) {
  const bool owner = (n < 15 && (n % 3) == 0) || n == 16;
  const int k = n == 16 ? 5 : n / 3;
#pragma unroll
  for (int t = 0; t < NT; ++t) {
    float tot[16];
#pragma unroll
    for (int r = 0; r < 16; ++r) {
      const float v = dm[t][r];
      const float v1 = __builtin_bit_cast(
          float, __builtin_amdgcn_update_dpp(0, __builtin_bit_cast(int, v), 0x101, 0xf, 0xf, true));
      const float v2 = __builtin_bit_cast(
          float, __builtin_amdgcn_update_dpp(0, __builtin_bit_cast(int, v), 0x102, 0xf, 0xf, true));
      tot[r] = (v + v1) + v2;
    }
#pragma unroll
    for (int r = 0; r < 16; ++r) dm[t][r] = 0.0f;
    if (owner && first) {
#pragma unroll
      for (int r = 0; r < 16; ++r) {
        const int j = t * 32 + (r & 3) + 8 * (r >> 2) + 4 * hf;
        acc64[j * stride + k] = (double)tot[r];
      }
    } else if (owner) {
#pragma unroll
      for (int r = 0; r < 16; ++r) {
        const int j = t * 32 + (r & 3) + 8 * (r >> 2) + 4 * hf;
        __hip_atomic_fetch_add(&acc64[j * stride + k], (double)tot[r], __ATOMIC_RELAXED, __HIP_MEMORY_SCOPE_WAVEFRONT);
      }
    }
  }
}


__device__ __forceinline__ double owner_sum(double v, int hf) {
  double s = hf == 0 ? v : 0.0;
#pragma unroll
  for (int m = 16; m > 0; m >>= 1) {
    const uint64_t bits = rl_f64_bits(s);
    const uint32_t lo = (uint32_t)__shfl_xor((int)(uint32_t)bits, m, 64);
    const uint32_t hi = (uint32_t)__shfl_xor((int)(uint32_t)(bits >> 32), m, 64);
    s = s + rl_f64_from_bits(((uint64_t)hi << 32) | lo);
  }
  return s;
}
__device__ __forceinline__ float half_sum(float v) {
#pragma unroll
  for (int m = 1; m < 32; m <<= 1) v = v + __shfl_xor(v, m, 64);
  return v;
}

template <int CHAIN, typename F>
__device__ __forceinline__ void load_weights(const uint32_t *__restrict__ wimg, int wave, int lane, int A, uint32_t *range,
                                             uint32_t *range_err, Frag (&fw)[NT][3], F fold) {
  const bool guard = blockIdx.x == 0 && wave == 0 && range != nullptr;
  float xmin = 0.0f, xmax = 0.0f;
  if (guard) range_bounds(range, lane, xmin, xmax);
#pragma unroll
  for (int t = 0; t < NT; ++t) {
    WRaw r;
    wimg_load(wimg, t, lane, fw[t], r, A);
    if (guard) range_guard_img(r, lane >> 5, xmin, xmax, range_err + CHAIN, range_veto(range, CHAIN));
    fold(t, r);
  }
}

struct Dealing {
  uint32_t share, first, n_waves;
};
template <int WAVES, int CHANNELS = 1>
__device__ __forceinline__ Dealing deal_tiles(int wave, uint32_t share_old, uint32_t share_young) {
  constexpr int WALKERS = WAVES / CHANNELS, HALF = WALKERS / 2;
  const int w = CHANNELS == 1 ? wave : wave & (WALKERS - 1);
  const uint32_t per_wg = HALF * (share_old + share_young);
  Dealing d;
  d.share = w < HALF ? share_old : share_young;
  d.first = blockIdx.x * per_wg +
            (w < HALF ? (uint32_t)w * share_old : HALF * share_old + (uint32_t)(w - HALF) * share_young);
  d.n_waves = gridDim.x * per_wg;
  return d;
}
template <bool TWO_BUFFERS, typename L, typename T>
__device__ __forceinline__ void walk_tiles(const Dealing &deal, uint32_t n_full, uint32_t tail, L &load_tile, T &tile) {
  const Dealing d = deal;
  for (uint32_t vw = 0; vw < d.share; ++vw) {
    const uint32_t wave_id = d.first + vw;
    if (wave_id < n_full) {
      auto op_a = load_tile(wave_id), op_b = op_a;
      if (!TWO_BUFFERS) {
        for (uint32_t g = wave_id; g < n_full; g += d.n_waves) {
          const uint32_t g1 = g + d.n_waves;
          op_b = load_tile(g1 < n_full ? g1 : g);
          tile(std::false_type{}, op_a, g);
          op_a = op_b;
        }
      } else {
        for (uint32_t g = wave_id; g < n_full; g += 2 * d.n_waves) {
          const uint32_t g1 = g + d.n_waves, g2 = g1 + d.n_waves;
          op_b = load_tile(g1 < n_full ? g1 : g);
          tile(std::false_type{}, op_a, g);
          if (g1 >= n_full) break;
          op_a = load_tile(g2 < n_full ? g2 : g1);
          tile(std::false_type{}, op_b, g1);
        }
      }
    }
    if (tail != 0 && n_full % d.n_waves == wave_id) tile(std::true_type{}, load_tile(n_full), n_full);
  }
}

template <int W, typename LIN>
__device__ __forceinline__ float transpose_sum(float (&ysh)[W][32][YROW], int w, const float (&yp)[16], LIN lin, int n,
                                               int hf) {
#pragma unroll
  for (int r = 0; r < 16; ++r) ysh[w][(r & 3) + 8 * (r >> 2) + 4 * hf][n] = yp[r];
  wave_lds_fence();
  float part = row_sum16v(&ysh[w][n][hf * 16]);
  part = part + lin();
  float p0, p1;
  both_halves(part, p0, p1);
  return p0 + p1;
}
__device__ __forceinline__ float linear_half(const float (&lv)[3], float xa, float xb, float xc, int hf) {
  float lin = lv[0] * xa;
  lin = __builtin_fmaf(lv[1], xb, lin);
  return __builtin_fmaf(lv[2], hf == 0 ? xc : 1.0f, lin);
}

template <int NW, int IMG>
__device__ __forceinline__ double image_sum(const double (*acc)[IMG], int src) {
  double s = acc[0][src];
#pragma unroll
  for (int w = 1; w < NW; ++w) s = s + acc[w][src];
  return s;
}
template <typename M>
__device__ __forceinline__ double dw2_sum(const float *__restrict__ W1, const float *__restrict__ b1, int j, M m) {
  double s = m(5) * (double)b1[j];
#pragma unroll
  for (int k = 0; k < PAR_D; ++k) s += m(k) * (double)W1[j * PAR_D + k];
  return s;
}
template <int CH, typename M, typename C>
__device__ __forceinline__ double grad_entry(uint32_t p, const float *__restrict__ params, M m, C coef) {
  const float *__restrict__ W1 = params, *__restrict__ b1 = params + PAR_B1;
  auto dw1 = [&](int j, int k) {
    double s = m(0, j, k) * coef(0, j);
    if (CH == 2) s = s + m(1, j, k) * coef(1, j);
    return s;
  };
  if (p < PAR_B1) return dw1((int)(p / (uint32_t)PAR_D), (int)(p % (uint32_t)PAR_D));
  if (p < PAR_W2) return dw1((int)(p - PAR_B1), 5);
  const int q = (int)(p - PAR_W2), a = q / PAR_H, j = q % PAR_H, c = CH == 1 ? 0 : a;
  return dw2_sum(W1, b1, j, [&](int k) { return m(c, j, k); });
}

}
```

### relearn_amd/csrc/engine.hpp

```cpp
#pragma once

#include <hip/hip_runtime.h>

#include <cstdint>
#include <cstdio>
#include <stdexcept>
#include <string>
#include <vector>

#include "../../include/relearn_hip.h"
#include "dev_mem.hpp"

struct RlError : std::runtime_error {
  int32_t code;
  RlError(int32_t c, const std::string &m) : std::runtime_error(m), code(c) {}
};

#define RL_HIP_CHECK(expr)                                                                          \
  do {                                                                                              \
    hipError_t _e = (expr);                                                                         \
    if (_e != hipSuccess)                                                                           \
      throw RlError(RL_ERR_HIP, std::string(#expr) + ": " + hipGetErrorString(_e) + " (" __FILE__ ":" + \
                                    std::to_string(__LINE__) + ")");                                \
  } while (0)

#define RL_REQUIRE(cond, msg)                                        \
  do {                                                               \
    if (!(cond)) throw RlError(RL_ERR_INVALID_ARGUMENT, (msg));      \
  } while (0)

struct CartPoleDev {
  double gravity, mass_pole, length_half_pole, friction_cart, friction_pole, time_step;
  double action_force, max_pos, max_angle;
  double total_weight, inv_total_mass, mass_length_pole;
  double init_low, init_scale;
  uint32_t key_env[8], key_actor[8];
  uint64_t lane_offset;
  uint32_t max_steps;
  int32_t limit_kind;
  uint32_t chain_size;
  uint32_t mem_actions;
  uint32_t bandit;
  float bandit_r[8];
  uint32_t meta_arms;
  int32_t meta_dist;
};

struct EnvStateDev {
  double *x, *xdot, *th, *thdot;
  uint8_t *nv_pos;
  uint32_t *steps_remaining;
  uint32_t *reset_count;
};

constexpr int RL_RANGE_WORDS = 2 * 64 * 32;
constexpr int RL_RANGE_ALLOC_WORDS = RL_RANGE_WORDS + 32;
constexpr int RL_GUARD_POLICY = 0, RL_GUARD_CRITIC = 1;
struct TrajDev {
  float *obs;
  uint8_t *action;
  float *reward;
  uint8_t *flag;
  float *term_obs;
  float *values;
  float *adv;
  float *rtg;
  float *tgt;
  uint32_t n, T, D;
  uint32_t *range;
  uint32_t *range_err;
};

struct alignas(32) ReplayRec {
  float x[5];
  float reward;
  uint32_t af;
  uint32_t pad;
};
struct alignas(32) ReplayNext {
  float x[8];
};
struct ReplayDev {
  ReplayRec *rec;
  ReplayNext *next;
  uint32_t *head, *count, *ep_head, *ep_count, *total;
  uint32_t *ep_end;
  uint64_t *actor_pos;
  int32_t *error;
  uint32_t N, C, E, D;
  float4 *hi;
};

struct DqnCountsDev {
  uint32_t n_eps, n_steps;
  int32_t error;
  uint32_t pad;
};

struct TrpoStateDev {
  float rr;
  int32_t cg_done;
  int32_t cg_iters;
  float loss0;
  float entropy;
  double step_size;
  int32_t ls_accepted;
  int32_t ls_index;
  double ls_ratio;
  float ls_loss, ls_kl;
  int32_t status;
  int32_t prev_saved;
};

struct LoopbackGroup;

constexpr int RL_IPC_MAX_RANKS = 16;

struct rl_engine {
  int device = -1;
  hipStream_t stream = nullptr;
  hipStream_t main_stream = nullptr, aux_stream = nullptr;
  hipEvent_t ev_fork = nullptr, ev_join = nullptr;
  int chan = 0;
  hipDeviceProp_t prop{};
  std::string last_error;
  hipEvent_t ev_begin = nullptr, ev_end = nullptr;
  bool profiling = false;
  double prof_ms[RL_K_CLASS_COUNT] = {0};
  uint64_t prof_launches[RL_K_CLASS_COUNT] = {0};
  std::vector<std::pair<int, std::pair<hipEvent_t, hipEvent_t>>> prof_pending;
  std::vector<hipEvent_t> prof_event_pool;
  void *comm = nullptr;
  void *comm_aux = nullptr;
  struct LoopbackGroup *loopback = nullptr;
  rl_host_allreduce_fn host_allreduce = nullptr;
  void *host_allreduce_ctx = nullptr;
  std::vector<float> host_allreduce_buf;
  float *ipc_box = nullptr;
  float *ipc_peer[RL_IPC_MAX_RANKS] = {nullptr};
  bool ipc_peer_local[RL_IPC_MAX_RANKS] = {false};
  int32_t *ipc_err = nullptr;
  uint32_t ipc_seq[2] = {0, 0};
  uint64_t ipc_timeout_ticks = 0;
  int ipc_box_ranks = 0, ipc_rank_of_box = -1;
  bool ipc_active = false;
  bool has_collective() const {
    return comm != nullptr || loopback != nullptr || host_allreduce != nullptr || ipc_active;
  }
  int rank = 0, n_ranks = 1;
  bool agreed_serial_env = false;
  void *pinned = nullptr;
  size_t pinned_bytes = 0;
  int64_t live_handles = 0;
  bool zombie = false;
  uint64_t call_epoch = 0;
  uint64_t error_epoch = 0;
  int kernel_variant = 0;
  bool serial_update = false;
  struct PendingUpdate {
    bool active = false, joined = false, collected = false;
    struct rl_traj *traj = nullptr;
    const struct rl_mlp *critic = nullptr;
    uint64_t steps = 0;
    rl_critic_stats stats{};
    std::vector<float> losses;
  } pending;
};

struct rl_env {
  rl_engine *eng;
  DevMem mem;
  rl_env_config cfg;
  int kind = RL_ENV_CARTPOLE;
  CartPoleDev dev;
  EnvStateDev st;
  uint32_t D, A;
  uint64_t t_global = 0;
  uint8_t *d_actions = nullptr, *d_flag = nullptr;
  float *d_reward = nullptr, *d_obs = nullptr, *d_term_obs = nullptr;
};

enum { RL_MODULE_MLP = 0, RL_MODULE_GRU_MLP = 1, RL_MODULE_LSTM_MLP = 2 };
inline bool rl_module_is_recurrent(int kind) { return kind == RL_MODULE_GRU_MLP || kind == RL_MODULE_LSTM_MLP; }
inline uint64_t rl_module_gates(int kind) { return kind == RL_MODULE_LSTM_MLP ? 4 : 3; }

constexpr uint32_t RL_MLP_MAX_HIDDEN = 4;
constexpr uint32_t RL_MLP_MAX_WIDTH = 256;
constexpr uint32_t RL_MLP_MAX_OUT = 8;
constexpr uint32_t RL_TRAJ_MAX_OBS_DIM = 8;
constexpr uint32_t RL_ENV_MIN_OBS_DIM = 4;
constexpr uint32_t RL_RNN_MAX_LAYERS = 4;

struct rl_mlp {
  rl_engine *eng;
  mutable DevMem mem;
  uint32_t in_dim, hidden, out_dim;
  uint64_t P;
  float *d_params = nullptr;
  mutable uint32_t *d_wimg = nullptr;
  mutable uint64_t wimg_epoch = 0;
  int kind = RL_MODULE_MLP;
  uint32_t gru_hidden = 0;
  uint32_t rnn_layers = 1;
  bool lane_kernels() const { return rnn_layers > 1 || in_dim > 5 || gru_hidden > 128 || hidden > 128 || !has_bias; }
  uint64_t rnn_layer_offset(uint32_t l) const {
    const uint64_t GH = rl_module_gates(kind) * (uint64_t)gru_hidden, nb = has_bias ? 2 * GH : 0;
    if (l == 0) return 0;
    return GH * (in_dim + gru_hidden) + nb + (uint64_t)(l - 1) * (GH * 2 * gru_hidden + nb);
  }
  uint32_t n_hidden = 1;
  uint32_t widths[RL_MLP_MAX_HIDDEN] = {0, 0, 0, 0};
  bool general = false;
  int act = 1, out_act = 0;
  rl_mlp *exec = nullptr;
  ~rl_mlp() { delete exec; }
  float *x_tmp = nullptr, *x_tan = nullptr;
  uint32_t n_layers() const { return n_hidden + 1; }
  uint32_t fan_in(uint32_t l) const { return l == 0 ? in_dim : widths[l - 1]; }
  uint32_t fan_out(uint32_t l) const { return l == n_hidden ? out_dim : widths[l]; }
  uint64_t layer_offset(uint32_t l) const {
    uint64_t o = 0;
    for (uint32_t i = 0; i < l; ++i) o += (uint64_t)fan_in(i) * fan_out(i) + (has_bias ? fan_out(i) : 0);
    return o;
  }
  bool has_bias = true;
  uint64_t bias_offset(uint32_t l) const { return has_bias ? layer_offset(l) + (uint64_t)fan_in(l) * fan_out(l) : P; }
  uint32_t hidden_units() const {
    uint32_t s = 0;
    for (uint32_t i = 0; i < n_hidden; ++i) s += widths[i];
    return s;
  }
};

struct SeqDev {
  float *act = nullptr;
  float *dpre = nullptr;
  float *out = nullptr;
  float *succ = nullptr;
  float *wg_slab = nullptr;
  uint32_t tiles = 0, chunks = 0, blocks_per_chunk = 0;
  struct Stack {
    float *st = nullptr;
    float *u = nullptr;
    float *z = nullptr;
    float *din = nullptr;
    float *dst = nullptr;
    float *rec = nullptr;
    float *a1 = nullptr;
    float *ur = nullptr;
    float *dg = nullptr;
    float *du = nullptr;
    uint32_t wg_rows = 0, wg_chunk = 0;
  } stack;
};

struct GenDev {
  float *act = nullptr, *tact = nullptr;
  float *delta = nullptr;
  float *z = nullptr, *tz = nullptr;
  int32_t *no_interrupt = nullptr;
};

enum : uint32_t {
  OPT_WEIGHT_DECAY = 1u,
  OPT_MOMENTUM = 2u,
  OPT_NESTEROV = 4u,
  OPT_CENTERED = 8u,
  OPT_FIRST_STEP = 16u,
};
struct OptStep {
  float neg_lr;
  float sqrt_bc2;
  float b1, b2, omb1, omb2;
  float eps, wd;
  float decay;
  float momentum, omd;
  float alpha, oma;
  uint32_t flags;
};
struct OptState {
  float *s0, *s1, *s2;
};

struct rl_adam {
  rl_engine *eng;
  DevMem mem;
  rl_mlp *mod;
  rl_optimizer_config cfg;
  float *d_state[3] = {nullptr, nullptr, nullptr};
  uint64_t *d_step = nullptr;
  uint64_t host_step = 0;
  uint64_t error_epoch = 0;
};

struct rl_traj {
  rl_engine *eng;
  DevMem mem;
  TrajDev d;
  uint64_t B;
  float *lp0 = nullptr;
  float *dz = nullptr;
  uint32_t act_planes = 2;
  uint32_t n_actions = 0, max_action = 0;
  double *slabA = nullptr;
  double *slabB = nullptr;
  float *vec = nullptr;
  float *cg_x = nullptr, *cg_r = nullptr, *cg_p = nullptr, *prev_params = nullptr, *descent = nullptr;
  float *td = nullptr;
  float *losses = nullptr;
  TrpoStateDev *trpo = nullptr;
  uint32_t nbA = 0, nbB = 0, nbV2 = 0, nbC = 0, Pmax = 0, max_losses = 0;
  uint32_t last_rows = 0;
  double *aux_slabA = nullptr, *aux_slabB = nullptr;
  float *aux_vec = nullptr;
  uint32_t aux_last_rows = 0;
  bool range_valid = false, range_fixed = false;
  bool range_reset = false;
  uint32_t *h_range_err = nullptr;
  bool guard_next_policy = true, guard_next_critic = true;
  bool rtg_scan_valid = false;
  float rtg_gamma = 0.0f;
  const float *last_targets = nullptr;
  uint32_t bwd_chunk = 0;
  SeqDev seq;
  GenDev gen;
};

struct rl_dqn {
  rl_engine *eng;
  DevMem mem;
  ~rl_dqn();
  rl_env *env;
  rl_mlp *qnet;
  rl_adam *opt;
  rl_dqn_config cfg;
  ReplayDev rp;
  uint64_t *d_agent_pos = nullptr;
  uint32_t *d_ep_lane = nullptr, *d_ep_start = nullptr, *d_ep_len = nullptr, *d_ep_off = nullptr;
  DqnCountsDev *d_counts = nullptr;
  uint8_t *d_flags = nullptr;
  uint64_t last_horizon = 0;
  uint32_t max_eps = 0;
  uint64_t max_steps_mb = 0;
  rl_traj *mb = nullptr;
  float *all_obs = nullptr, *all_target = nullptr;
  uint8_t *all_action = nullptr, *all_flag = nullptr;
  bool td_in_kernel = false;
  hipStream_t draw_stream = nullptr;
  std::vector<hipEvent_t> draw_events;
  hipEvent_t main_event = nullptr;
  DqnCountsDev *h_counts = nullptr;
  float *d_q = nullptr, *d_q_next = nullptr;
  float *snap = nullptr;
  float *own_obs = nullptr, *own_target = nullptr;
  uint8_t *own_action = nullptr, *own_flag = nullptr;
  uint64_t global_steps = 0;
  uint64_t steps_per_lane = 0;
  uint32_t last_n_eps = 0, last_n_steps = 0, last_batch_index = 0;
  uint64_t last_total_steps = 0;
};

struct ProfScope {
  rl_engine *e;
  int cls;
  hipEvent_t a = nullptr, b = nullptr;
  ProfScope(rl_engine *eng, int c);
  ~ProfScope();
};

void rl_allreduce_sum_f32(rl_engine *e, float *d_buf, size_t count);
void comm_agree(rl_engine *e);
bool ipc_allreduce_fits(const rl_engine *e, size_t count);
void ipc_allreduce(rl_engine *e, float *d_buf, size_t count);
void ipc_check(rl_engine *e);
void ipc_teardown(rl_engine *e);
```

### relearn_amd/csrc/kernels.hpp

```cpp
#pragma once
#include <cstdlib>
#include <functional>
#define RL_SEQ_ACT_ARRAYS 9
#define RL_SEQ_DPRE_ARRAYS 6
#include "engine.hpp"

void launch_env_reset(rl_env *env);
void launch_env_observe(rl_env *env, float *d_obs);
void launch_env_step(rl_env *env);
void launch_rollout(rl_env *env, const rl_mlp *policy, rl_traj *traj);
void launch_values(rl_traj *traj, const rl_mlp *critic);
void launch_gae(rl_traj *traj, const rl_mlp *critic, float gamma, float lambda);
void launch_value_targets(rl_traj *traj, const rl_mlp *critic, float gamma);
void launch_mlp_forward_host_rows(rl_mlp *mlp, const float *d_in_soa, size_t rows, float *d_out_soa);
void launch_obs_range(rl_traj *traj);
inline void traj_ensure_range(rl_traj *traj) {
  if (traj->range_valid || traj->range_fixed) return;
  launch_obs_range(traj);
  traj->range_valid = true;
}
inline bool fused_5_128_fits(const rl_traj *t, const rl_mlp *m, uint32_t out_dim, bool offsets = true) {
  return m->kind == RL_MODULE_MLP && !m->general && t->d.D == 5 && m->hidden == 128 && m->out_dim == out_dim &&
         (!offsets || (uint64_t)(t->d.T + 1) * t->d.n * 5 < (1ull << 30));
}
inline uint32_t fused_grid(const rl_traj *t, uint32_t walkers) {
  const uint64_t n_tiles = (t->B + 31) / 32, cus = (uint64_t)t->eng->prop.multiProcessorCount;
  const uint64_t nb = (n_tiles + walkers - 1) / walkers;
  return (uint32_t)(nb > cus ? cus : nb);
}
inline TrajDev fused_traj_dev(const rl_traj *t, bool &guard_next) {
  TrajDev d = t->d;
  if (!guard_next) d.range = nullptr;
  guard_next = false;
  return d;
}

const uint32_t *wimg_ensure(const rl_mlp *m);
inline uint32_t *wimg_if_current(const rl_mlp *m) {
  return m->d_wimg != nullptr && m->wimg_epoch == m->eng->call_epoch ? m->d_wimg : nullptr;
}
inline void wimg_invalidate(const rl_mlp *m) { m->wimg_epoch = 0; }

inline void seq_ensure_outputs(rl_traj *t) {
  const uint64_t B = (uint64_t)t->d.T * t->d.n;
  t->mem.ensure(t->seq.out, 2 * B);
  t->mem.ensure(t->seq.succ, 2 * B);
}

enum PolicyPassMode { PASS_INIT = 0, PASS_EVAL = 1, PASS_JVP = 2, PASS_DQN = 3, PASS_PPO = 4 };
void launch_policy_pass(rl_traj *traj, const rl_mlp *policy, int mode, const float *d_tangent, uint64_t B_total,
                        const int32_t *d_skip_flag, float clip_lo = 0.0f, float clip_hi = 0.0f);
void launch_critic_fwd(rl_traj *traj, const rl_mlp *critic, uint64_t B_total);
void launch_mlp_backward(rl_traj *traj, const rl_mlp *mlp, const int32_t *d_skip_flag);
void launch_reduce(rl_traj *traj, uint32_t P, bool useA, bool useB, uint32_t rowsA, uint32_t rowsB);

void launch_trpo_begin(rl_traj *traj, rl_mlp *policy, uint64_t B_total);
void launch_cg_step(rl_traj *traj, uint32_t P, float reg, float tol);
void launch_cg_finish(rl_traj *traj, uint32_t P);
void launch_step_size(rl_traj *traj, rl_mlp *policy, float reg, double max_kl);
void launch_ls_set_params(rl_traj *traj, rl_mlp *policy, double ratio);
void launch_ls_check(rl_traj *traj, uint32_t P, uint64_t B_total, int index, double ratio, double max_kl);
void launch_ls_finalize(rl_traj *traj, rl_mlp *policy, double max_kl, int accept_violation);
void launch_adam_step(rl_traj *traj, rl_adam *opt, int loss_slot, uint64_t B_total);
void launch_adam_step_vec(rl_adam *opt, const float *d_grad);
void launch_reduce_adam(rl_traj *traj, rl_adam *opt, uint32_t rowsA, uint32_t rowsB, int loss_slot, uint64_t B_total);

bool launch_critic_step_v2(rl_traj *traj, const rl_mlp *critic, uint64_t B_total);
bool launch_policy_v2(rl_traj *traj, const rl_mlp *policy, int mode, const float *d_tangent, uint64_t B_total,
                      const int32_t *d_skip_flag, float clip_lo = 0.0f, float clip_hi = 0.0f);

void launch_rollout_dqn(rl_env *env, const rl_mlp *qnet, const ReplayDev &rp, uint32_t T, uint64_t p_int,
                        int always_explore, uint8_t *d_flags, uint32_t *d_range = nullptr);
void launch_rollout_dqn_general(rl_env *env, const rl_mlp *qnet, rl_traj *ws, float *d_q, const ReplayDev &rp, uint32_t T,
                                uint64_t p_int, int always_explore, uint8_t *d_flags);
void launch_dqn_td_targets(rl_engine *eng, float *d_target, const uint8_t *d_flag, const float *d_q_next, uint32_t n,
                           float gamma);
struct AgentKey { uint32_t w[8]; };
void launch_dqn_sample(rl_engine *eng, hipStream_t stream, const ReplayDev &rp, const AgentKey &key, uint64_t *d_agent_pos,
                       uint32_t minibatch_steps, uint32_t max_eps, uint32_t *d_lane, uint32_t *d_start,
                       uint32_t *d_len, uint32_t *d_off, DqnCountsDev *d_counts, int sequential,
                       uint32_t n_batches = 1);
void launch_dqn_build_all(rl_engine *eng, const ReplayDev &rp, uint32_t n_batches, uint32_t widest_eps, uint32_t max_eps,
                          const uint32_t *d_lane, const uint32_t *d_start, const uint32_t *d_len, const uint32_t *d_off,
                          const DqnCountsDev *d_counts, float *d_obs, size_t obs_stride, uint8_t *d_action,
                          float *d_target, size_t step_stride, float gamma, uint8_t *d_flag);
void launch_replay_planes(rl_engine *eng, const ReplayDev &rp, int field, void *d_out);
bool launch_dqn_step_bf16(rl_traj *mb, const rl_mlp *qnet, uint64_t B_total, float gamma);
bool launch_dqn_step_pair(rl_traj *mb, const rl_mlp *qnet, uint64_t B_total);
void launch_dqn_build_minibatch(rl_engine *eng, const ReplayDev &rp, uint32_t n_eps, const uint32_t *d_lane,
                                const uint32_t *d_start, const uint32_t *d_len, const uint32_t *d_off,
                                float *d_obs, size_t out_plane, uint8_t *d_action, float *d_target, float gamma,
                                int one_step_td, const rl_mlp *qnet);

void launch_rollout_gru(rl_env *env, const rl_mlp *policy, rl_traj *traj);
void launch_rollout_chain_mlp(rl_env *env, const rl_mlp *policy, rl_traj *traj);
void launch_gru_seq_forward(rl_traj *traj, const rl_mlp *mod, float *d_out, float *d_succ, float *d_act,
                            const int32_t *d_skip = nullptr);
void gen_ensure(rl_traj *t, const rl_mlp *m, uint64_t rows, bool tangent, bool backward);
void launch_gen_forward(rl_traj *t, const rl_mlp *m, const float *x, size_t x_stride, uint64_t rows, float *out);
void launch_gen_policy_pass(rl_traj *t, const rl_mlp *m, int mode, const float *d_tangent, uint64_t B_total,
                            const int32_t *d_skip, float clip_lo, float clip_hi);
void launch_gen_critic_fwd(rl_traj *t, const rl_mlp *m, uint64_t B_total);
void launch_gen_backward(rl_traj *t, const rl_mlp *m, const int32_t *d_skip);
void traj_ensure_slabs(rl_traj *t, uint64_t rowsA, uint64_t P, uint64_t rowsB);
void traj_ensure_action_planes(rl_traj *t, uint32_t n_actions);
constexpr int RL_GEN_CRITIC = 100;
bool gen_mfma_fits(const rl_traj *t, const rl_mlp *m);
bool launch_gen_mfma(rl_traj *t, const rl_mlp *m, int mode, const float *d_tangent, uint64_t B_total,
                     const int32_t *d_skip, float clip_lo, float clip_hi);
void launch_gen_values(rl_traj *t, const rl_mlp *critic);
void launch_gen_rollout(rl_env *env, const rl_mlp *policy, rl_traj *t);
void launch_rollout_stepwise(rl_env *env, rl_traj *t, const float *z, const std::function<void(uint32_t)> &forward);
void launch_gen_wgrad_planes(rl_traj *t, const float *dY, size_t dys, int N, const float *X, size_t xs, int K, size_t S,
                             uint32_t chunk, uint32_t rows, uint32_t P, uint32_t offW, uint32_t offB,
                             const int32_t *d_skip);
void stack_ensure(rl_traj *t, const rl_mlp *mod, bool training);
void launch_stack_rollout(rl_env *env, const rl_mlp *policy, rl_traj *traj);
void launch_stack_forward(rl_traj *traj, const rl_mlp *mod, float *d_out, float *d_succ, bool record,
                          const int32_t *d_skip);
void launch_stack_backward(rl_traj *traj, const rl_mlp *mod, const int32_t *d_skip);
void launch_stack_tangent(rl_traj *traj, const rl_mlp *mod, const float *d_tangent, const int32_t *d_skip);
void launch_seq_pad(const rl_mlp *real, float *exec_dst, const float *real_src);
void launch_seq_unpad(const rl_mlp *real, const float *exec_src, float *real_dst);
void launch_gru_train_forward(rl_traj *traj, const rl_mlp *mod, float *d_out, float *d_act, const int32_t *d_skip);
void launch_lstm_train_forward(rl_traj *traj, const rl_mlp *mod, float *d_out, float *d_act, const int32_t *d_skip);
void launch_seq_train_head_forward(rl_traj *traj, const rl_mlp *mod, float *d_out, float *d_act, const int32_t *d_skip);
void launch_gru_train_head_backward(rl_traj *traj, const rl_mlp *mod, float *d_slab, const int32_t *d_skip);
void launch_gru_train_recur_backward(rl_traj *traj, const rl_mlp *mod, const int32_t *d_skip);
void launch_gru_train_wgrad(rl_traj *traj, const rl_mlp *mod, const int32_t *d_skip);
constexpr uint32_t RL_SEQ_HEAD_ROWS = 512;
void launch_seq_gae(rl_traj *traj, float gamma, float lambda);
void launch_seq_value_targets(rl_traj *traj, float gamma);
void launch_seq_policy_dlogits(rl_traj *traj, int mode, uint64_t B_total, float clip_lo, float clip_hi,
                               const int32_t *d_skip = nullptr);
void launch_seq_critic_dvalues(rl_traj *traj, uint64_t B_total);
void launch_gru_backward(rl_traj *traj, const rl_mlp *mod, const int32_t *d_skip = nullptr);
void launch_gru_tangent(rl_traj *traj, const rl_mlp *mod, const float *d_tangent, uint64_t B_total,
                        const int32_t *d_skip);
```

### relearn_amd/csrc/kernels_mfma.hip

```cpp
#include <type_traits>

#include "bf16_tile.hpp"
#include "device_fns.hpp"
#include "kernels.hpp"
#include "policy_fast.hpp"

constexpr int V2_WAVES = 8;

constexpr int PB_FLUSH = 16;

template <int MODE, int WAVES, bool FW_LDS = false>
__global__ void __launch_bounds__(WAVES * 64)
    k_policy_bf16(TrajDev tr, const float *__restrict__ params, const uint32_t *__restrict__ wimg,
                  const float *__restrict__ tangent, float *__restrict__ lp0, double *__restrict__ slabA,
                  double *__restrict__ slabB, float inv_B, uint32_t P, const int32_t *__restrict__ skip, float clip_lo,
                  float clip_hi, uint32_t share_old, uint32_t share_young) {
  using bt::Frag;
  constexpr int D = 5, H = 128, NT = bt::NT, A = 2;
  constexpr bool BWD = MODE != PASS_EVAL;
  constexpr bool JVP = MODE == PASS_JVP;
  constexpr int IW = 7;
  constexpr int PIMG_M = H * IW + 5;
  __shared__ __attribute__((aligned(16))) float Ysh[JVP ? 1 : WAVES][32][bt::YROW];
  __shared__ double Acc[WAVES][BWD ? PIMG_M : 4];
  __shared__ uint4 Fz[JVP ? bt::L2_KS : 1][64];
  __shared__ uint4 Fw[FW_LDS ? NT * 3 : 1][64];
  if (skip != nullptr && *skip != 0) return;

  const int lane = threadIdx.x & 63;
  const int wave = __builtin_amdgcn_readfirstlane((int)(threadIdx.x >> 6));
  const int n = lane & 31, hf = lane >> 5;
  const float *__restrict__ W1 = params, *__restrict__ b1 = W1 + bt::PAR_B1, *__restrict__ W2 = params + bt::PAR_W2,
                           *__restrict__ b2 = params + bt::par_b2(A);
  const size_t B = (size_t)tr.T * tr.n;
  const size_t plane = (size_t)(tr.T + 1) * tr.n;
  double *acc64 = Acc[wave];
  bool flushed = false;

  Frag fw[NT][3];
  float w2d[NT];
  float lvd[3] = {0.0f, 0.0f, 0.0f};
  float tb2d = 0.0f;
  bt::load_weights<bt::GUARD_POLICY>(wimg, wave, lane, 2, tr.range, tr.range_err, fw, [&](int t, const bt::WRaw &r) {
    if (FW_LDS && wave == t) {
#pragma unroll
      for (int i = 0; i < 3; ++i) Fw[t * 3 + i][lane] = fw[t][i].x;
    }
    const float wd = r.w2[0] - r.w2[1];
    if (!JVP) {
      lvd[0] = __builtin_fmaf(wd, r.wa, lvd[0]);
      lvd[1] = __builtin_fmaf(wd, r.wb, lvd[1]);
      lvd[2] = __builtin_fmaf(wd, r.wc, lvd[2]);
    }
    w2d[t] = bt::FWD_UNSCALE * wd;
  });
  if (JVP) {
    const float *__restrict__ V1 = tangent, *__restrict__ vb1 = V1 + bt::PAR_B1, *__restrict__ V2 = tangent + bt::PAR_W2;
    bt::l2_build(Fz, (int)threadIdx.x, WAVES * 64, [&](int j, int k) {
      const float wd = W2[j] - W2[H + j], t2d = V2[j] - V2[H + j];
      const float w = k < D ? W1[j * D + k] : b1[j], v = k < D ? V1[j * D + k] : vb1[j];
      return __builtin_fmaf(t2d, w, wd * v);
    });
  }
  if (JVP || FW_LDS) __syncthreads();
  if (JVP) {
    const float *__restrict__ vb2 = tangent + bt::par_b2(A);
    tb2d = vb2[0] - vb2[1];
  } else {
#pragma unroll
    for (int q = 0; q < 3; ++q) lvd[q] = bt::half_sum(lvd[q]);
  }
  const float b2d = b2[0] - b2[1];
  Frag selb[2], idb[2];
  if (BWD) bt::sel_frags(lane, selb);
  if (JVP) bt::ident_frags(lane, idb);
  bt::f32x16 dm[NT];
#pragma unroll
  for (int t = 0; t < NT; ++t) dm[t] = (bt::f32x16){0, 0, 0, 0, 0, 0, 0, 0, 0, 0, 0, 0, 0, 0, 0, 0};
  double sum0 = 0.0, sum1 = 0.0, sum2 = 0.0, db2_0 = 0.0, db2_1 = 0.0;
  float s0f = 0.0f, s1f = 0.0f, s2f = 0.0f, d0f = 0.0f, d1f = 0.0f;
  auto fold = [&]() {
    sum0 += (double)s0f;
    sum1 += (double)s1f;
    sum2 += (double)s2f;
    db2_0 += (double)d0f;
    db2_1 += (double)d1f;
    s0f = s1f = s2f = d0f = d1f = 0.0f;
  };
  bt::wave_lds_fence();

  const uint32_t B32 = (uint32_t)B, plane32 = (uint32_t)plane;
  const uint32_t n_full = B32 / 32u, tail = B32 & 31u;
  if (WAVES != 8) share_old = share_young = 1u;
  const bt::Dealing deal = bt::deal_tiles<WAVES>(wave, share_old, share_young);
  const bt::rsrc_t obs_r = bt::make_rsrc(tr.obs, (uint32_t)D * plane32 * 4u), lp0_r = bt::make_rsrc(lp0, 2u * B32 * 4u);
  const bt::rsrc_t adv_r = bt::make_rsrc(tr.adv, B32 * 4u), act_r = bt::make_rsrc(tr.action, B32);
  const uint32_t off_a = ((uint32_t)(2 * hf) * plane32 + (uint32_t)n) * 4u, off_b = off_a + plane32 * 4u;
  const uint32_t off_c = (4u * plane32 + (uint32_t)n) * 4u, off_s = (uint32_t)n * 4u, off_s1 = off_s + B32 * 4u;
  int since_flush = 0;
  struct TileOp {
    float xa, xb, xc, l0, l1, adv;
    int act;
  };
  auto load_tile = [&](uint32_t g) {
    TileOp o;
    const uint32_t soff = g * 128u;
    o.xa = bt::buf_f32(obs_r, off_a, soff);
    o.xb = bt::buf_f32(obs_r, off_b, soff);
    o.xc = bt::buf_f32(obs_r, off_c, soff);
    o.l0 = o.l1 = o.adv = 0.0f;
    o.act = 0;
    if (MODE != PASS_INIT) {
      o.l0 = bt::buf_f32(lp0_r, off_s, soff);
      o.l1 = bt::buf_f32(lp0_r, off_s1, soff);
    }
    if (!JVP) {
      o.adv = bt::buf_f32(adv_r, off_s, soff);
      o.act = (int)bt::buf_u8(act_r, (uint32_t)n, g * 32u);
    }
    return o;
  };
  auto tile = [&](auto ragged, TileOp op_in, uint32_t g) {
    constexpr bool RAGGED = decltype(ragged)::value;
    struct {
      float xa, xb, xc, l0, l1, adv;
      int act;
      bool valid;
    } op;
    op.valid = RAGGED ? (uint32_t)n < tail : true;
    op.xa = op.valid ? op_in.xa : 0.0f;
    op.xb = op.valid ? op_in.xb : 0.0f;
    op.xc = op.valid ? op_in.xc : 0.0f;
    op.l0 = op.valid ? op_in.l0 : 0.0f;
    op.l1 = op.valid ? op_in.l1 : 0.0f;
    op.adv = op.valid ? op_in.adv : 0.0f;
    op.act = op.valid ? op_in.act : 0;
    const size_t sidx = (size_t)g * 32 + n;
    Frag fa[3];
    bt::input_frags(op.xa, op.xb, op.xc, op.valid, hf, fa);
    Frag ga[NT][2];
    float y0[16];
#pragma unroll
    for (int r = 0; r < 16; ++r) y0[r] = 0.0f;
    bt::f32x16 q = {0, 0, 0, 0, 0, 0, 0, 0, 0, 0, 0, 0, 0, 0, 0, 0};
    auto fwd = [&](int t) {
      if (FW_LDS) {
        Frag f[3];
#pragma unroll
        for (int i = 0; i < 3; ++i) f[i].x = Fw[t * 3 + i][lane];
        return bt::layer1(fa, f);
      }
      return bt::layer1(fa, fw[t]);
    };
    bt::f32x16 c = fwd(0);
#pragma unroll
    for (int t = 0; t < NT; ++t) {
      bt::f32x16 cn = c;
      if (t + 1 < NT) cn = fwd(t + 1);
      if (!JVP) {
#pragma unroll
        for (int r = 0; r < 16; ++r) y0[r] = __builtin_fmaf(__builtin_fabsf(c[r]), w2d[t], y0[r]);
      }
      if (BWD) bt::mask_tile(c, ga[t]);
      if (JVP) q = bt::masked_sum_tile(ga[t], idb, Fz, t, lane, q);
      c = cn;
    }
    float s0;
    if (JVP) {
      float p0, p1;
      bt::both_halves(bt::l2_dot(q, op.xa, op.xb, hf == 0 ? op.xc : 1.0f), p0, p1);
      s0 = p0 + p1;
    } else {
      s0 = 0.5f * bt::transpose_sum(
                      Ysh, JVP ? 0 : wave, y0, [&] { return bt::linear_half(lvd, op.xa, op.xb, op.xc, hf); }, n, hf);
      bt::wave_lds_fence();
    }
    float dz0 = 0.0f, dz1 = 0.0f;
    if (JVP) {
      const float delta = s0 + tb2d;
      const SoftPair old = soft_pair(op.l0 - op.l1);
      dz0 = op.valid ? (old.p[0] * old.p[1]) * delta * inv_B : 0.0f;
      dz1 = -dz0;
    } else {
      const float adv = op.adv;
      const int act = op.act;
      const SoftPair sp = soft_pair(s0 + b2d);
      const float(&lp)[2] = sp.lp;
      if (MODE == PASS_PPO) {
        const float l0a = act == 0 ? op.l0 : op.l1;
        const float lpa = act == 0 ? lp[0] : lp[1];
        const float ratio = fast_expf(lpa - l0a);
        const float clipped = ratio < clip_lo ? clip_lo : (ratio > clip_hi ? clip_hi : ratio);
        const float u1 = ratio * adv, u2 = clipped * adv;
        const bool inside = ratio >= clip_lo && ratio <= clip_hi;
        const float gr = u1 < u2 ? adv : (u1 > u2 ? (inside ? adv : 0.0f) : (inside ? adv : 0.5f * adv));
        const float cc = -(gr * ratio) * inv_B;
        dz0 = op.valid ? cc * ((act == 0 ? 1.0f : 0.0f) - sp.p[0]) : 0.0f;
        dz1 = op.valid ? cc * ((act == 1 ? 1.0f : 0.0f) - sp.p[1]) : 0.0f;
        if (op.valid) s0f = s0f + (u1 < u2 ? u1 : u2);
      } else if (MODE == PASS_INIT) {
        if (op.valid && hf == 0) {
          lp0[sidx] = lp[0];
          lp0[B + sidx] = lp[1];
        }
        const float lpa = act == 0 ? lp[0] : lp[1];
        const float ratio = fast_expf(lpa - lpa);
        const float cc = -(ratio * adv) * inv_B;
        const float pa0 = sp.p[0], pa1 = sp.p[1];
        dz0 = op.valid ? cc * ((act == 0 ? 1.0f : 0.0f) - pa0) : 0.0f;
        dz1 = op.valid ? cc * ((act == 1 ? 1.0f : 0.0f) - pa1) : 0.0f;
        const float cl0 = lp[0] < -3.402823466e+38f ? -3.402823466e+38f : lp[0];
        const float cl1 = lp[1] < -3.402823466e+38f ? -3.402823466e+38f : lp[1];
        float ent = cl0 * pa0;
        ent += cl1 * pa1;
        if (op.valid) {
          s0f = __builtin_fmaf(ratio, adv, s0f);
          s1f = s1f - ent;
          s2f = __builtin_fmaf(lpa, adv, s2f);
        }
      } else {
        const float l00 = op.l0, l01 = op.l1;
        const float lpa = act == 0 ? lp[0] : lp[1];
        const float l0a = act == 0 ? l00 : l01;
        const float ratio = fast_expf(lpa - l0a);
        float rel0 = l00 - lp[0], rel1 = l01 - lp[1];
        if (rel0 < -3.402823466e+38f) rel0 = -3.402823466e+38f;
        if (rel1 < -3.402823466e+38f) rel1 = -3.402823466e+38f;
        const SoftPair old = soft_pair(l00 - l01);
        float kl = rel0 * old.p[0];
        kl += rel1 * old.p[1];
        if (op.valid) {
          s0f = __builtin_fmaf(ratio, adv, s0f);
          s1f = s1f + kl;
        }
      }
    }
    if (BWD) {
      d0f = d0f + dz0;
      d1f = d1f + dz1;
      Frag ub[2];
      bt::piece_frags_mfma(0.5f * (dz0 - dz1), op.xa, op.xb, op.xc, hf, selb, ub);
      bt::backward(ga, ub, dm);
      if (++since_flush == PB_FLUSH) {
        since_flush = 0;
        bt::flush(dm, acc64, IW, n, hf, !flushed);
        flushed = true;
        fold();
      }
    } else if (++since_flush == PB_FLUSH) {
      since_flush = 0;
      fold();
    }
  };
  bt::walk_tiles<!JVP>(deal, n_full, tail, load_tile, tile);
  if (BWD && (since_flush != 0 || !flushed)) bt::flush(dm, acc64, IW, n, hf, !flushed);
  fold();
  const double r0 = bt::owner_sum(sum0, hf), r1 = bt::owner_sum(sum1, hf);
  const double r2 = bt::owner_sum(db2_0, hf), r3 = bt::owner_sum(db2_1, hf);
  const double r4 = MODE == PASS_INIT ? bt::owner_sum(sum2, hf) : 0.0;
  constexpr int TAIL = BWD ? H * IW : 0;
  if (lane == 0) {
    if (BWD) {
      acc64[TAIL + 0] = r2;
      acc64[TAIL + 1] = r3;
      acc64[TAIL + 2] = r0;
      acc64[TAIL + 3] = r1;
      if (MODE == PASS_INIT) acc64[TAIL + 4] = r4;
    } else {
      acc64[0] = r0;
      acc64[1] = r1;
    }
  }
  __syncthreads();
  auto tot = [&](int src) { return bt::image_sum<WAVES>(Acc, src); };
  if (BWD) {
    for (uint32_t p = threadIdx.x; p < P; p += WAVES * 64) {
      double s;
      if (p < bt::par_b2(A)) {
        s = bt::grad_entry<1>(p, params, [&](int, int j, int k) { return tot(j * IW + k); },
                              [&](int, int j) { return (double)W2[j] - (double)W2[H + j]; });
        if (p >= bt::PAR_W2 + H) s = -s;
      } else {
        s = tot(TAIL + (int)(p - bt::par_b2(A)));
      }
      slabA[(size_t)blockIdx.x * P + p] = s;
    }
  }
  if (threadIdx.x < 4) {
    double v = 0.0;
    if (BWD) {
      if (!JVP && threadIdx.x < 2) v = tot(TAIL + 2 + threadIdx.x);
      if (MODE == PASS_INIT && threadIdx.x == 2) v = tot(TAIL + 4);
    } else if (threadIdx.x < 2) {
      v = tot(threadIdx.x);
    }
    slabB[(size_t)blockIdx.x * 4 + threadIdx.x] = v;
  }
}

bool launch_policy_v2(rl_traj *traj, const rl_mlp *policy, int mode, const float *d_tangent, uint64_t B_total,
                      const int32_t *d_skip, float clip_lo, float clip_hi) {
  if (policy->general) return launch_gen_mfma(traj, policy, mode, d_tangent, B_total, d_skip, clip_lo, clip_hi);
  if (!fused_5_128_fits(traj, policy, 2)) return false;
  if (mode == PASS_DQN) return false;
  traj_ensure_range(traj);
  const uint32_t *wimg = wimg_ensure(policy);
  ProfScope ps(traj->eng, mode == PASS_JVP ? RL_K_POLICY_FVP : RL_K_POLICY_FUSED);
  float inv_B = 1.0f / (float)B_total;
  traj->nbV2 = fused_grid(traj, V2_WAVES);
  traj->last_rows = traj->nbV2;
  dim3 g(traj->nbV2), b(V2_WAVES * 64);
  hipStream_t s = traj->eng->stream;
  uint32_t P = (uint32_t)policy->P;
  const TrajDev d = fused_traj_dev(traj, traj->guard_next_policy);
#define BLAUNCH(MM)                                                                                                  \
  hipLaunchKernelGGL((k_policy_bf16<MM, V2_WAVES>), g, b, 0, s, d, policy->d_params, wimg, d_tangent, traj->lp0,       \
                     traj->slabA, traj->slabB, inv_B, P, d_skip, clip_lo, clip_hi, bt::SHARE_OLD, bt::SHARE_YOUNG)
  if (mode == PASS_INIT) BLAUNCH(PASS_INIT);
  else if (mode == PASS_JVP) BLAUNCH(PASS_JVP);
  else if (mode == PASS_PPO) BLAUNCH(PASS_PPO);
  else {
    constexpr int EVAL_WAVES = 16;
    hipLaunchKernelGGL((k_policy_bf16<PASS_EVAL, EVAL_WAVES, true>), g, dim3(EVAL_WAVES * 64), 0, s, d,
                       policy->d_params, wimg, d_tangent, traj->lp0, traj->slabA, traj->slabB, inv_B, P, d_skip, clip_lo,
                       clip_hi, 1u, 1u);
  }
#undef BLAUNCH
  return true;
}
```

### relearn_amd/csrc/kernels_update.hip

```cpp
#include "bf16_tile.hpp"
#include "comm_ipc.hpp"
#include "device_fns.hpp"
#include "kernels.hpp"
#include "policy_terms.hpp"

#include <cfloat>
#include <cmath>

static inline uint32_t cdiv(size_t a, size_t b) { return (uint32_t)((a + b - 1) / b); }

template <int D, int MODE>
__global__ void __launch_bounds__(256) k_policy_pass(TrajDev tr, const float *__restrict__ params,
                                                     const float *__restrict__ tangent, int H,
                                                     float *__restrict__ lp0, float *__restrict__ dz,
                                                     double *__restrict__ slabB, float inv_B,
                                                     const int32_t *__restrict__ skip, float clip_lo,
                                                     float clip_hi) {
  constexpr int A = 2;
  __shared__ double red[256];
  if (skip != nullptr && *skip != 0) return;
  const size_t B = (size_t)tr.T * tr.n;
  const size_t plane = (size_t)(tr.T + 1) * tr.n;
  double s0 = 0.0, s1 = 0.0, s2 = 0.0;
  for (size_t b = (size_t)blockIdx.x * 256 + threadIdx.x; b < B; b += (size_t)gridDim.x * 256) {
// ... 595 lines not shown
  const int c = lane & (CW - 1), rg = w * GPW + lane / CW;
  const uint32_t p = blockIdx.x * CW + (uint32_t)c;
  const uint32_t vetoed = veto != nullptr ? *veto : 0u;
  float p_old = 0.0f, s0 = 0.0f, s1 = 0.0f, s2 = 0.0f;
  if (threadIdx.x < CW && p < P) {
    p_old = params[p];
    if (opt_has_slot<RULE>(0, k.flags)) s0 = st.s0[p];
    if (opt_has_slot<RULE>(1, k.flags)) s1 = st.s1[p];
    if (opt_has_slot<RULE>(2, k.flags)) s2 = st.s2[p];
  }
  auto partial = [&](const double *__restrict__ slab, uint32_t nb, uint32_t stride, uint32_t col) {
    constexpr int U = 256 / RG;
    double acc = 0.0;
    for (uint32_t r0 = (uint32_t)rg; r0 < nb; r0 += RG * U) {
      double x[U];
#pragma unroll
      for (int u = 0; u < U; ++u) {
        const uint32_t r = r0 + RG * u;
        x[u] = r < nb ? slab[(size_t)r * stride + col] : 0.0;
      }
#pragma unroll
      for (int u = 0; u < U; ++u) acc = acc + x[u];
    }
    return acc;
  };
  double acc = 0.0;
  if (p < P) acc = partial(slabA, nbA, P, p);
  else if (p < P + 4) acc = partial(slabB, nbB, 4, p - P);
  part[rg][c] = acc;
  __syncthreads();
  if (threadIdx.x >= CW || p >= P + 4) return;
  double t = part[0][c];
#pragma unroll
  for (int r = 1; r < RG; ++r) t = t + part[r][c];
  const float gsum = (float)t;
  vec[p] = gsum;
  if (p >= P) {
    if (p == P && loss_out) *loss_out = (float)((double)gsum * inv_B);
    return;
  }
  if (vetoed != 0u) return;
  if (p == 0) *step_ptr = step;
  const float w_new = opt_apply<RULE>(p_old, gsum, s0, s1, s2, k);
  if (opt_has_slot<RULE>(0, k.flags)) st.s0[p] = s0;
  if (opt_has_slot<RULE>(1, k.flags)) st.s1[p] = s1;
  if (opt_has_slot<RULE>(2, k.flags)) st.s2[p] = s2;
  params[p] = w_new;
  if (wimg) bt::wimg_store_param(wimg, p, w_new, A);
}

static const int32_t *comm_err_word(const rl_engine *e) { return e->ipc_active ? e->ipc_err : (const int32_t *)nullptr; }
static const uint32_t *veto_word(const rl_traj *traj, const rl_mlp *m) {
  if (traj->d.range == nullptr) return nullptr;
  return traj->d.range + RL_RANGE_WORDS + (m->out_dim == 1 ? RL_GUARD_CRITIC : RL_GUARD_POLICY);
}

void launch_policy_pass(rl_traj *traj, const rl_mlp *policy, int mode, const float *d_tangent, uint64_t B_total,
                        const int32_t *d_skip, float clip_lo, float clip_hi) {
  ProfScope ps(traj->eng, RL_K_POLICY_PASS);
  RL_REQUIRE(policy->out_dim == 2 || policy->general, "policy pass: the fused kernels are built for 2-action policies");
  if (policy->general) return launch_gen_policy_pass(traj, policy, mode, d_tangent, B_total, d_skip, clip_lo, clip_hi);
  float inv_B = 1.0f / (float)B_total;
  dim3 g(traj->nbB), b(256);
  hipStream_t s = traj->eng->stream;
  int H = (int)policy->hidden;
#define PASS(DD, MM)                                                                                           \
  hipLaunchKernelGGL((k_policy_pass<DD, MM>), g, b, 0, s, traj->d, policy->d_params, d_tangent, H, traj->lp0, \
                     traj->dz, traj->slabB, inv_B, d_skip, clip_lo, clip_hi)
  if (mode == PASS_DQN) inv_B = 2.0f / (float)B_total;
  if (traj->d.D == 5) {
    if (mode == PASS_INIT) PASS(5, PASS_INIT);
    else if (mode == PASS_EVAL) PASS(5, PASS_EVAL);
    else if (mode == PASS_DQN) PASS(5, PASS_DQN);
    else if (mode == PASS_PPO) PASS(5, PASS_PPO);
    else PASS(5, PASS_JVP);
  } else {
    if (mode == PASS_INIT) PASS(4, PASS_INIT);
    else if (mode == PASS_EVAL) PASS(4, PASS_EVAL);
    else if (mode == PASS_DQN) PASS(4, PASS_DQN);
    else if (mode == PASS_PPO) PASS(4, PASS_PPO);
    else PASS(4, PASS_JVP);
  }
#undef PASS
}

void launch_critic_fwd(rl_traj *traj, const rl_mlp *critic, uint64_t B_total) {
  ProfScope ps(traj->eng, RL_K_CRITIC_FWD);
  if (critic->general) return launch_gen_critic_fwd(traj, critic, B_total);
  float two_over_B = 2.0f / (float)B_total;
  dim3 g(traj->nbB), b(256);
  if (traj->d.D == 5)
    hipLaunchKernelGGL(k_critic_fwd<5>, g, b, 0, traj->eng->stream, traj->d, critic->d_params, (int)critic->hidden,
                       traj->dz, traj->slabB, two_over_B);
  else
    hipLaunchKernelGGL(k_critic_fwd<4>, g, b, 0, traj->eng->stream, traj->d, critic->d_params, (int)critic->hidden,
                       traj->dz, traj->slabB, two_over_B);
}

void launch_mlp_backward(rl_traj *traj, const rl_mlp *mlp, const int32_t *d_skip) {
  ProfScope ps(traj->eng, RL_K_BACKWARD);
  if (mlp->general) return launch_gen_backward(traj, mlp, d_skip);
  RL_REQUIRE(mlp->hidden <= 128, "backward kernel v1 supports hidden <= 128");
  dim3 g(traj->nbA), b(128);
  size_t plane = (size_t)(traj->d.T + 1) * traj->d.n;
  hipStream_t s = traj->eng->stream;
  uint32_t P = (uint32_t)mlp->P;
#define BWD(DD, AA)                                                                                            \
  hipLaunchKernelGGL((k_mlp_backward<DD, AA>), g, b, 0, s, mlp->d_params, (int)mlp->hidden, traj->d.obs, plane, \
                     traj->dz, (size_t)traj->B, traj->bwd_chunk, traj->slabA, P, d_skip)
  if (traj->d.D == 5 && mlp->out_dim == 2) BWD(5, 2);
  else if (traj->d.D == 5 && mlp->out_dim == 1) BWD(5, 1);
  else if (traj->d.D == 4 && mlp->out_dim == 2) BWD(4, 2);
  else if (traj->d.D == 4 && mlp->out_dim == 1) BWD(4, 1);
  else throw RlError(RL_ERR_UNSUPPORTED, "backward: unsupported (obs_dim, out_dim)");
#undef BWD
}

static int reduce_width(uint32_t P) { return P + 4 > 2048 ? 64 : 16; }

void launch_reduce(rl_traj *traj, uint32_t P, bool useA, bool useB, uint32_t rowsA, uint32_t rowsB) {
  ProfScope ps(traj->eng, RL_K_REDUCE);
  if (reduce_width(P) == 64)
    hipLaunchKernelGGL(k_reduce, dim3(cdiv(P + 4, 64)), dim3(1024), 0, traj->eng->stream, traj->slabA, rowsA, P,
                       traj->slabB, rowsB, traj->vec, useA ? 1 : 0, useB ? 1 : 0);
  else
    hipLaunchKernelGGL(k_reduce_narrow<16>, dim3(cdiv(P + 4, 16)), dim3(1024), 0, traj->eng->stream, traj->slabA, rowsA,
                       P, traj->slabB, rowsB, traj->vec, useA ? 1 : 0, useB ? 1 : 0);
}

void launch_trpo_begin(rl_traj *traj, rl_mlp *policy, uint64_t B_total) {
  ProfScope ps(traj->eng, RL_K_SMALL);
  hipLaunchKernelGGL(k_trpo_begin, dim3(1), dim3(SB), 0, traj->eng->stream, traj->vec, (uint32_t)policy->P,
                     1.0 / (double)B_total, traj->cg_x, traj->cg_r, traj->cg_p, traj->trpo);
}

void launch_cg_step(rl_traj *traj, uint32_t P, float reg, float tol) {
  ProfScope ps(traj->eng, RL_K_SMALL);
  hipLaunchKernelGGL(k_cg_step, dim3(1), dim3(SB), 0, traj->eng->stream, traj->vec, P, reg, tol, traj->cg_x,
                     traj->cg_r, traj->cg_p, traj->trpo);
}

void launch_cg_finish(rl_traj *traj, uint32_t P) {
  ProfScope ps(traj->eng, RL_K_SMALL);
  hipLaunchKernelGGL(k_cg_finish, dim3(1), dim3(SB), 0, traj->eng->stream, traj->cg_x, P);
}

void launch_step_size(rl_traj *traj, rl_mlp *policy, float reg, double max_kl) {
  ProfScope ps(traj->eng, RL_K_SMALL);
  hipLaunchKernelGGL(k_step_size, dim3(1), dim3(SB), 0, traj->eng->stream, traj->vec, (uint32_t)policy->P, reg,
                     max_kl, traj->cg_x, traj->descent, policy->d_params, traj->prev_params, traj->trpo);
}

void launch_ls_set_params(rl_traj *traj, rl_mlp *policy, double ratio) {
  ProfScope ps(traj->eng, RL_K_SMALL);
  hipLaunchKernelGGL(k_ls_set_params, dim3(1), dim3(SB), 0, traj->eng->stream, policy->d_params, traj->prev_params,
                     traj->descent, (uint32_t)policy->P, (float)ratio, traj->trpo, comm_err_word(traj->eng),
                     wimg_if_current(policy), (int)policy->out_dim);
}

const uint32_t *wimg_ensure(const rl_mlp *m) {
  rl_engine *e = m->eng;
  if (m->d_wimg == nullptr) {
    RL_HIP_CHECK(hipSetDevice(e->device));
    m->d_wimg = m->mem.alloc<uint32_t>(bt::WIMG_WORDS);
    m->wimg_epoch = 0;
  }
  if (m->wimg_epoch != e->call_epoch) {
    ProfScope ps(e, RL_K_SMALL);
    hipLaunchKernelGGL(k_wimg_build, dim3(((uint32_t)m->P + SB - 1) / SB), dim3(SB), 0, e->stream, m->d_params,
                       (uint32_t)m->P, m->d_wimg, (int)m->out_dim);
    m->wimg_epoch = e->call_epoch;
  }
  return m->d_wimg;
}

void launch_ls_check(rl_traj *traj, uint32_t P, uint64_t B_total, int index, double ratio, double max_kl) {
  ProfScope ps(traj->eng, RL_K_SMALL);
  hipLaunchKernelGGL(k_ls_check, dim3(1), dim3(64), 0, traj->eng->stream, traj->vec, P, 1.0 / (double)B_total, index,
                     ratio, max_kl, traj->trpo);
}

void launch_ls_finalize(rl_traj *traj, rl_mlp *policy, double max_kl, int accept_violation) {
  ProfScope ps(traj->eng, RL_K_SMALL);
  hipLaunchKernelGGL(k_ls_finalize, dim3(1), dim3(SB), 0, traj->eng->stream, policy->d_params, traj->prev_params,
                     (uint32_t)policy->P, max_kl, accept_violation, traj->trpo, comm_err_word(traj->eng),
                     veto_word(traj, policy));
  wimg_invalidate(policy);
}

static OptStep adam_next_step(rl_adam *opt) {
  if (opt->error_epoch != opt->eng->error_epoch) {
    rl_engine *e = opt->eng;
    RL_HIP_CHECK(hipStreamSynchronize(e->main_stream));
    RL_HIP_CHECK(hipStreamSynchronize(e->aux_stream));
    uint64_t s = 0;
    RL_HIP_CHECK(hipMemcpyAsync(&s, opt->d_step, sizeof(s), hipMemcpyDeviceToHost, e->stream));
    RL_HIP_CHECK(hipStreamSynchronize(e->stream));
    opt->host_step = s;
    opt->error_epoch = e->error_epoch;
  }
  opt->host_step += 1;
  const rl_optimizer_config &c = opt->cfg;
  OptStep k{};
  k.eps = (float)c.eps;
  k.wd = (float)c.weight_decay;
  if (c.weight_decay != 0.0) k.flags |= OPT_WEIGHT_DECAY;
  if (c.kind == RL_OPTIMIZER_ADAM || c.kind == RL_OPTIMIZER_ADAMW) {
    const double bc1 = 1.0 - std::pow(c.beta1, (double)opt->host_step);
    const double bc2 = 1.0 - std::pow(c.beta2, (double)opt->host_step);
    k.neg_lr = -(float)(c.learning_rate / bc1);
    k.sqrt_bc2 = (float)std::sqrt(bc2);
    k.b1 = (float)c.beta1;
    k.b2 = (float)c.beta2;
    k.omb1 = (float)(1.0 - c.beta1);
    k.omb2 = (float)(1.0 - c.beta2);
    k.decay = (float)(1.0 - c.learning_rate * c.weight_decay);
  } else {
    k.neg_lr = (float)(-c.learning_rate);
    k.momentum = (float)c.momentum;
    k.omd = (float)(1.0 - c.dampening);
    k.alpha = (float)c.alpha;
    k.oma = (float)(1.0 - c.alpha);
    if (c.kind == RL_OPTIMIZER_SGD ? c.momentum != 0.0 : c.momentum > 0.0) k.flags |= OPT_MOMENTUM;
    if (c.kind == RL_OPTIMIZER_SGD && c.nesterov) k.flags |= OPT_NESTEROV;
    if (c.kind == RL_OPTIMIZER_RMSPROP && c.centered) k.flags |= OPT_CENTERED;
    if (opt->host_step == 1) k.flags |= OPT_FIRST_STEP;
  }
  return k;
}

#define RL_WITH_RULE(KIND, CALL)                                                      \
  switch (KIND) {                                                                     \
    case RL_OPTIMIZER_ADAM: { constexpr int RULE = RL_OPTIMIZER_ADAM; CALL; } break;   \
    case RL_OPTIMIZER_ADAMW: { constexpr int RULE = RL_OPTIMIZER_ADAMW; CALL; } break; \
    case RL_OPTIMIZER_SGD: { constexpr int RULE = RL_OPTIMIZER_SGD; CALL; } break;     \
    case RL_OPTIMIZER_RMSPROP: { constexpr int RULE = RL_OPTIMIZER_RMSPROP; CALL; } break; \
    default: throw RlError(RL_ERR_INVALID_ARGUMENT, "optimizer: unknown kind");       \
  }

void launch_reduce_adam(rl_traj *traj, rl_adam *opt, uint32_t rowsA, uint32_t rowsB, int loss_slot,
                        uint64_t B_total) {
  ProfScope ps(traj->eng, RL_K_REDUCE);
  uint32_t P = (uint32_t)opt->mod->P;
  rl_engine *e = traj->eng;
  RL_REQUIRE(!e->ipc_active || opt->cfg.kind == RL_OPTIMIZER_ADAM,
             "the exchange inside the reduction launch is built for Adam only");
  const OptStep k = adam_next_step(opt);
  const OptState st{opt->d_state[0], opt->d_state[1], opt->d_state[2]};
  float *loss_out = loss_slot >= 0 ? traj->losses + loss_slot : (float *)nullptr;
  if (e->ipc_active) {
    ProfScope pa(e, RL_K_ALLREDUCE);
    const IpcPeers peers = ipc_peers_next(e);
    hipLaunchKernelGGL((k_reduce_opt<RL_OPTIMIZER_ADAM, true>), dim3(cdiv(P + 4, 64)), dim3(1024), 0, e->stream,
                       traj->slabA, rowsA, P, traj->slabB, rowsB, traj->vec, opt->mod->d_params, st, opt->d_step,
                       opt->host_step, k, 1.0 / (double)B_total, loss_out, peers, wimg_if_current(opt->mod),
                       (int)opt->mod->out_dim, veto_word(traj, opt->mod));
  } else if (reduce_width(P) != 64) {
    RL_WITH_RULE(opt->cfg.kind,
                 hipLaunchKernelGGL((k_reduce_opt_narrow<RULE, 16>), dim3(cdiv(P + 4, 16)), dim3(1024), 0, e->stream,
                                    traj->slabA, rowsA, P, traj->slabB, rowsB, traj->vec, opt->mod->d_params, st,
                                    opt->d_step, opt->host_step, k, 1.0 / (double)B_total, loss_out,
                                    wimg_if_current(opt->mod), (int)opt->mod->out_dim, veto_word(traj, opt->mod)));
  } else {
    RL_WITH_RULE(opt->cfg.kind,
                 hipLaunchKernelGGL((k_reduce_opt<RULE, false>), dim3(cdiv(P + 4, 64)), dim3(1024), 0, e->stream,
                                    traj->slabA, rowsA, P, traj->slabB, rowsB, traj->vec, opt->mod->d_params, st,
                                    opt->d_step, opt->host_step, k, 1.0 / (double)B_total, loss_out, IpcPeers{},
                                    wimg_if_current(opt->mod), (int)opt->mod->out_dim, veto_word(traj, opt->mod)));
  }
}

static void launch_opt_step(rl_adam *opt, hipStream_t stream, const float *d_grad, const float *loss_sum, double inv_B,
                            float *loss_out, const int32_t *comm_err, const uint32_t *veto) {
  uint32_t P = (uint32_t)opt->mod->P;
  const OptStep k = adam_next_step(opt);
  const OptState st{opt->d_state[0], opt->d_state[1], opt->d_state[2]};
  RL_WITH_RULE(opt->cfg.kind,
               hipLaunchKernelGGL(k_opt_step<RULE>, dim3((P + SB - 1) / SB), dim3(SB), 0, stream, opt->mod->d_params,
                                  d_grad, st, opt->d_step, P, opt->host_step, k, loss_sum, inv_B, loss_out, comm_err,
                                  wimg_if_current(opt->mod), (int)opt->mod->out_dim, veto));
}

void launch_adam_step(rl_traj *traj, rl_adam *opt, int loss_slot, uint64_t B_total) {
  ProfScope ps(traj->eng, RL_K_SMALL);
  uint32_t P = (uint32_t)opt->mod->P;
  launch_opt_step(opt, traj->eng->stream, traj->vec, traj->vec + P, 1.0 / (double)B_total,
                  loss_slot >= 0 ? traj->losses + loss_slot : (float *)nullptr, comm_err_word(traj->eng),
                  veto_word(traj, opt->mod));
}

void launch_adam_step_vec(rl_adam *opt, const float *d_grad) {
  ProfScope ps(opt->mod->eng, RL_K_SMALL);
  launch_opt_step(opt, opt->mod->eng->stream, d_grad, (const float *)nullptr, 0.0, (float *)nullptr,
                  (const int32_t *)nullptr, (const uint32_t *)nullptr);
}
```

Baseline: 498.5 million env-steps/s.

## Cache ReLU masks from policy init pass as fp4 image for CG Fisher-vector passes

The TRPO init pass now stores the per-sample hidden-layer ReLU masks, packed to fp4 with the hardware conversion builtins, into a per-trajectory mask image. The Jacobian-vector passes used in the 10 CG iterations read this image back instead of reloading weights and recomputing the first-layer forward. They also use a deeper load-ahead tile walker to hide the extra memory reads. This trades recomputing the layer-1 MFMA work on every FVP for extra global traffic and a large buffer, with a fallback to recomputation if allocation fails or the parameters change.

```diff
diff --git a/include/relearn_hip.h b/include/relearn_hip.h
--- a/include/relearn_hip.h
+++ b/include/relearn_hip.h
@@ -258,6 +258,8 @@
 int32_t rl_actor_critic_update_finish(rl_traj *traj, rl_critic_stats *critic_stats ,
                                       float *critic_losses_out );
 int32_t rl_engine_set_serial_update(rl_engine *engine, int32_t serial);
+enum { RL_FVP_DEFAULT = 0, RL_FVP_RECOMPUTE = 1, RL_FVP_MASK_IMAGE = 2 };
+int32_t rl_engine_set_fvp_form(rl_engine *engine, int32_t form);
 
 typedef struct {
   uint64_t opt_steps_per_update;
diff --git a/relearn_amd/__init__.py b/relearn_amd/__init__.py
--- a/relearn_amd/__init__.py
+++ b/relearn_amd/__init__.py
@@ -25,6 +25,7 @@
 (TRAJ_OBS, TRAJ_ACTION, TRAJ_REWARD, TRAJ_FLAG, TRAJ_TERM_OBS, TRAJ_VALUES, TRAJ_ADVANTAGES,
  TRAJ_RETURNS, TRAJ_TARGETS) = range(9)
 VALUE_TARGET_REWARD_TO_GO, VALUE_TARGET_ONE_STEP_TD = 0, 1
+FVP_DEFAULT, FVP_RECOMPUTE, FVP_MASK_IMAGE = 0, 1, 2
 OPTIMIZER_ADAM, OPTIMIZER_ADAMW, OPTIMIZER_SGD, OPTIMIZER_RMSPROP = 0, 1, 2, 3
 KERNEL_CLASSES = ["env_step", "rollout", "values", "gae", "policy_pass", "backward", "reduce", "small",
                   "critic_fwd", "allreduce", "critic_fused", "policy_fused", "policy_fvp"]
@@ -45,7 +46,7 @@
     "rl_adam_config_default", "rl_adam_create", "rl_adam_destroy", "rl_adam_step_host",
     "rl_optimizer_config_default", "rl_optimizer_create", "rl_optimizer_step_host", "rl_optimizer_state_read",
     "rl_critic_update", "rl_critic_gradient", "rl_values_opt_config_default", "rl_values_opt_update",
-    "rl_actor_critic_update", "rl_actor_critic_update_begin", "rl_actor_critic_update_finish", "rl_engine_set_serial_update",
+    "rl_actor_critic_update", "rl_actor_critic_update_begin", "rl_actor_critic_update_finish", "rl_engine_set_serial_update", "rl_engine_set_fvp_form",
     "rl_ppo_config_default", "rl_ppo_update", "rl_reinforce_update", "rl_reward_to_go",
     "rl_actor_to_cbor", "rl_module_from_cbor", "rl_tensor_def_to_cbor", "rl_tensor_def_from_cbor",
     "rl_indexed_type_space_to_cbor",
@@ -238,6 +239,9 @@
     def set_serial_update(self, serial):
         _check(lib().rl_engine_set_serial_update(self.h, C.c_int32(1 if serial else 0)), self.h)
 
+    def set_fvp_form(self, form):
+        _check(lib().rl_engine_set_fvp_form(self.h, C.c_int32(form)), self.h)
+
     def timer_begin(self):
         _check(lib().rl_timer_begin(self.h), self.h)
 
diff --git a/relearn_amd/csrc/abi.hip b/relearn_amd/csrc/abi.hip
--- a/relearn_amd/csrc/abi.hip
+++ b/relearn_amd/csrc/abi.hip
@@ -346,6 +346,14 @@
     RL_REQUIRE(e, "engine is NULL");
     RL_REQUIRE(variant == 0 || variant == 1, "kernel variant must be 0 (best) or 1 (v1 reference kernels)");
     e->kernel_variant = variant;
+  });
+}
+
+int32_t rl_engine_set_fvp_form(rl_engine *e, int32_t form) {
+  return guarded(e, [&] {
+    RL_REQUIRE(e, "engine is NULL");
+    RL_REQUIRE(form >= RL_FVP_DEFAULT && form <= RL_FVP_MASK_IMAGE, "Fisher-vector form must be one of RL_FVP_*");
+    e->fvp_form = form;
   });
 }
 
diff --git a/relearn_amd/csrc/abi_internal.hpp b/relearn_amd/csrc/abi_internal.hpp
--- a/relearn_amd/csrc/abi_internal.hpp
+++ b/relearn_amd/csrc/abi_internal.hpp
@@ -102,6 +102,7 @@
   const float *tangent = nullptr;
   const int32_t *skip = nullptr;
   float clip_lo = 0.0f, clip_hi = 0.0f;
+  bool keep_masks = false;
   bool forward_only = false;
   bool reduce = true;
   uint64_t B_total = 0;
diff --git a/relearn_amd/csrc/abi_update.hip b/relearn_amd/csrc/abi_update.hip
--- a/relearn_amd/csrc/abi_update.hip
+++ b/relearn_amd/csrc/abi_update.hip
@@ -65,7 +65,7 @@
   bool fused = false;
   if (traj->eng->kernel_variant == 0) {
     if (row.fused == FUSED_POLICY)
-      fused = launch_policy_v2(traj, mod, req.kind, req.tangent, Bt, req.skip, req.clip_lo, req.clip_hi);
+      fused = launch_policy_v2(traj, mod, req.kind, req.tangent, Bt, req.skip, req.clip_lo, req.clip_hi, req.keep_masks);
     else if (row.fused == FUSED_CRITIC)
       fused = launch_critic_step_v2(traj, mod, Bt);
   }
@@ -124,7 +124,9 @@
   uint32_t P = (uint32_t)policy->P;
   uint64_t Bt = b_total(traj);
   float reg = (float)cfg->hpv_reg_coeff;
-  run_pass(policy, traj, RUN_INIT);
+  PassRequest init(RUN_INIT);
+  init.keep_masks = true;
+  run_pass(policy, traj, init);
   launch_trpo_begin(traj, policy, Bt);
   PassRequest fvp(RUN_JVP);
   fvp.tangent = traj->cg_p;
@@ -215,7 +217,9 @@
     check_policy(policy, traj);
     RL_REQUIRE(v && out, "NULL argument");
     uint32_t P = (uint32_t)policy->P;
-    run_pass(policy, traj, RUN_INIT);
+    PassRequest init(RUN_INIT);
+    init.keep_masks = true;
+    run_pass(policy, traj, init);
     h2d(traj->eng, traj->cg_x, v, P * sizeof(float));
     PassRequest fvp(RUN_JVP);
     fvp.tangent = traj->cg_x;
diff --git a/relearn_amd/csrc/bf16_tile.hpp b/relearn_amd/csrc/bf16_tile.hpp
--- a/relearn_amd/csrc/bf16_tile.hpp
+++ b/relearn_amd/csrc/bf16_tile.hpp
@@ -262,6 +262,41 @@
 #pragma unroll
     for (int i = 0; i < 4; ++i)
       ga[s].u[i] = mask_pair(s + i == 0 ? first : c[8 * s + 2 * i], c[8 * s + 2 * i + 1], first);
+}
+
+typedef uint32_t u32x4 __attribute__((ext_vector_type(4)));
+constexpr uint32_t MIMG_TILE_BYTES = 2u * 64u * 16u;
+constexpr uint32_t MIMG_TILE_UINT4 = 2u * 64u;
+constexpr int MIMG_AUX = 2;
+__device__ __forceinline__ uint32_t mask_squeeze(const Frag &g) {
+  uint32_t w = 0u;
+  w = __builtin_amdgcn_cvt_scalef32_pk_fp4_bf16(w, __builtin_bit_cast(bf16x2, g.u[0]), 1.0f, 0);
+  w = __builtin_amdgcn_cvt_scalef32_pk_fp4_bf16(w, __builtin_bit_cast(bf16x2, g.u[1]), 1.0f, 1);
+  w = __builtin_amdgcn_cvt_scalef32_pk_fp4_bf16(w, __builtin_bit_cast(bf16x2, g.u[2]), 1.0f, 2);
+  w = __builtin_amdgcn_cvt_scalef32_pk_fp4_bf16(w, __builtin_bit_cast(bf16x2, g.u[3]), 1.0f, 3);
+  return w;
+}
+__device__ __forceinline__ void mask_unsqueeze(uint32_t w, Frag &g) {
+  g.u[0] = __builtin_bit_cast(uint32_t, __builtin_amdgcn_cvt_scalef32_pk_bf16_fp4(w, 1.0f, 0));
+  g.u[1] = __builtin_bit_cast(uint32_t, __builtin_amdgcn_cvt_scalef32_pk_bf16_fp4(w, 1.0f, 1));
+  g.u[2] = __builtin_bit_cast(uint32_t, __builtin_amdgcn_cvt_scalef32_pk_bf16_fp4(w, 1.0f, 2));
+  g.u[3] = __builtin_bit_cast(uint32_t, __builtin_amdgcn_cvt_scalef32_pk_bf16_fp4(w, 1.0f, 3));
+}
+__device__ __forceinline__ void mimg_store_half(rsrc_t r, int lane, uint32_t g, int half, const Frag (&ga)[NT][2]) {
+  u32x4 v;
+#pragma unroll
+  for (int w = 0; w < 4; ++w) v[w] = mask_squeeze(ga[2 * half + (w >> 1)][w & 1]);
+  __builtin_amdgcn_raw_buffer_store_b128(v, r, lane * 16 + half * 1024, (int)(g * MIMG_TILE_BYTES), MIMG_AUX);
+}
+__device__ __forceinline__ u32x4 mimg_load(rsrc_t r, int lane, uint32_t g, int half) {
+  return __builtin_amdgcn_raw_buffer_load_b128(r, lane * 16 + half * 1024, (int)(g * MIMG_TILE_BYTES), MIMG_AUX);
+}
+__device__ __forceinline__ void mimg_unpack(const u32x4 &lo, const u32x4 &hi, Frag (&ga)[NT][2]) {
+#pragma unroll
+  for (int w = 0; w < 4; ++w) {
+    mask_unsqueeze(lo[w], ga[w >> 1][w & 1]);
+    mask_unsqueeze(hi[w], ga[2 + (w >> 1)][w & 1]);
+  }
 }
 
 constexpr int L2_KS = 8;
@@ -467,6 +502,35 @@
   }
 }
 
+template <int AHEAD, typename L, typename T>
+__device__ __forceinline__ void walk_tiles_ahead(const Dealing &deal, uint32_t n_full, uint32_t tail, L &load_tile, T &tile) {
+  const Dealing d = deal;
+  for (uint32_t vw = 0; vw < d.share; ++vw) {
+    const uint32_t wave_id = d.first + vw;
+    if (wave_id < n_full) {
+      decltype(load_tile(0u)) op[AHEAD + 1];
+#pragma unroll
+      for (int j = 0; j < AHEAD; ++j) {
+        const uint32_t gj = wave_id + (uint32_t)j * d.n_waves;
+        op[j] = load_tile(gj < n_full ? gj : wave_id);
+      }
+      op[AHEAD] = op[0];
+      [&] {
+        for (uint32_t g = wave_id;; g += (uint32_t)(AHEAD + 1) * d.n_waves) {
+#pragma unroll
+          for (int j = 0; j <= AHEAD; ++j) {
+            const uint32_t gj = g + (uint32_t)j * d.n_waves, gl = gj + (uint32_t)AHEAD * d.n_waves;
+            if (gj >= n_full) return;
+            op[(j + AHEAD) % (AHEAD + 1)] = load_tile(gl < n_full ? gl : gj);
+            tile(std::false_type{}, op[j], gj);
+          }
+        }
+      }();
+    }
+    if (tail != 0 && n_full % d.n_waves == wave_id) tile(std::true_type{}, load_tile(n_full), n_full);
+  }
+}
+
 template <int W, typename LIN>
 __device__ __forceinline__ float transpose_sum(float (&ysh)[W][32][YROW], int w, const float (&yp)[16], LIN lin, int n,
                                                int hf) {
diff --git a/relearn_amd/csrc/engine.hpp b/relearn_amd/csrc/engine.hpp
--- a/relearn_amd/csrc/engine.hpp
+++ b/relearn_amd/csrc/engine.hpp
@@ -157,6 +157,7 @@
   uint64_t error_epoch = 0;
   int kernel_variant = 0;
   bool serial_update = false;
+  int fvp_form = 0;
   struct PendingUpdate {
     bool active = false, joined = false, collected = false;
     struct rl_traj *traj = nullptr;
@@ -320,6 +321,10 @@
   bool guard_next_policy = true, guard_next_critic = true;
   bool rtg_scan_valid = false;
   float rtg_gamma = 0.0f;
+  uint4 *mimg = nullptr;
+  uint64_t mimg_epoch = 0;
+  const rl_mlp *mimg_policy = nullptr;
+  bool mimg_unavailable = false;
   const float *last_targets = nullptr;
   uint32_t bwd_chunk = 0;
   SeqDev seq;
diff --git a/relearn_amd/csrc/kernels.hpp b/relearn_amd/csrc/kernels.hpp
--- a/relearn_amd/csrc/kernels.hpp
+++ b/relearn_amd/csrc/kernels.hpp
@@ -41,6 +41,10 @@
 }
 inline void wimg_invalidate(const rl_mlp *m) { m->wimg_epoch = 0; }
 
+inline bool mimg_valid(const rl_traj *t, const rl_mlp *m) {
+  return t->mimg != nullptr && t->mimg_policy == m && t->mimg_epoch == t->eng->call_epoch;
+}
+
 inline void seq_ensure_outputs(rl_traj *t) {
   const uint64_t B = (uint64_t)t->d.T * t->d.n;
   t->mem.ensure(t->seq.out, 2 * B);
@@ -67,7 +71,7 @@
 
 bool launch_critic_step_v2(rl_traj *traj, const rl_mlp *critic, uint64_t B_total);
 bool launch_policy_v2(rl_traj *traj, const rl_mlp *policy, int mode, const float *d_tangent, uint64_t B_total,
-                      const int32_t *d_skip_flag, float clip_lo = 0.0f, float clip_hi = 0.0f);
+                      const int32_t *d_skip_flag, float clip_lo = 0.0f, float clip_hi = 0.0f, bool keep_masks = false);
 
 void launch_rollout_dqn(rl_env *env, const rl_mlp *qnet, const ReplayDev &rp, uint32_t T, uint64_t p_int,
                         int always_explore, uint8_t *d_flags, uint32_t *d_range = nullptr);
diff --git a/relearn_amd/csrc/kernels_mfma.hip b/relearn_amd/csrc/kernels_mfma.hip
--- a/relearn_amd/csrc/kernels_mfma.hip
+++ b/relearn_amd/csrc/kernels_mfma.hip
@@ -7,18 +7,22 @@
 
 constexpr int V2_WAVES = 8;
 
+constexpr int MIMG_AHEAD = 3;
 constexpr int PB_FLUSH = 16;
 
-template <int MODE, int WAVES, bool FW_LDS = false>
+template <int MODE, int WAVES, bool FW_LDS = false, bool MASKS = false>
 __global__ void __launch_bounds__(WAVES * 64)
     k_policy_bf16(TrajDev tr, const float *__restrict__ params, const uint32_t *__restrict__ wimg,
                   const float *__restrict__ tangent, float *__restrict__ lp0, double *__restrict__ slabA,
                   double *__restrict__ slabB, float inv_B, uint32_t P, const int32_t *__restrict__ skip, float clip_lo,
-                  float clip_hi, uint32_t share_old, uint32_t share_young) {
+                  float clip_hi, uint32_t share_old, uint32_t share_young, uint4 *mimg) {
   using bt::Frag;
   constexpr int D = 5, H = 128, NT = bt::NT, A = 2;
   constexpr bool BWD = MODE != PASS_EVAL;
   constexpr bool JVP = MODE == PASS_JVP;
+  constexpr bool CACHED = JVP && MASKS;
+  constexpr bool KEEP = MODE == PASS_INIT && MASKS;
+  static_assert(!MASKS || JVP || MODE == PASS_INIT, "PASS_INIT writes the mask image, PASS_JVP reads it");
   constexpr int IW = 7;
   constexpr int PIMG_M = H * IW + 5;
   __shared__ __attribute__((aligned(16))) float Ysh[JVP ? 1 : WAVES][32][bt::YROW];
@@ -41,19 +45,21 @@
   float w2d[NT];
   float lvd[3] = {0.0f, 0.0f, 0.0f};
   float tb2d = 0.0f;
-  bt::load_weights<bt::GUARD_POLICY>(wimg, wave, lane, 2, tr.range, tr.range_err, fw, [&](int t, const bt::WRaw &r) {
-    if (FW_LDS && wave == t) {
-#pragma unroll
-      for (int i = 0; i < 3; ++i) Fw[t * 3 + i][lane] = fw[t][i].x;
-    }
-    const float wd = r.w2[0] - r.w2[1];
-    if (!JVP) {
-      lvd[0] = __builtin_fmaf(wd, r.wa, lvd[0]);
-      lvd[1] = __builtin_fmaf(wd, r.wb, lvd[1]);
-      lvd[2] = __builtin_fmaf(wd, r.wc, lvd[2]);
-    }
-    w2d[t] = bt::FWD_UNSCALE * wd;
-  });
+  if (!CACHED) {
+    bt::load_weights<bt::GUARD_POLICY>(wimg, wave, lane, 2, tr.range, tr.range_err, fw, [&](int t, const bt::WRaw &r) {
+      if (FW_LDS && wave == t) {
+#pragma unroll
+        for (int i = 0; i < 3; ++i) Fw[t * 3 + i][lane] = fw[t][i].x;
+      }
+      const float wd = r.w2[0] - r.w2[1];
+      if (!JVP) {
+        lvd[0] = __builtin_fmaf(wd, r.wa, lvd[0]);
+        lvd[1] = __builtin_fmaf(wd, r.wb, lvd[1]);
+        lvd[2] = __builtin_fmaf(wd, r.wc, lvd[2]);
+      }
+      w2d[t] = bt::FWD_UNSCALE * wd;
+    });
+  }
   if (JVP) {
     const float *__restrict__ V1 = tangent, *__restrict__ vb1 = V1 + bt::PAR_B1, *__restrict__ V2 = tangent + bt::PAR_W2;
     bt::l2_build(Fz, (int)threadIdx.x, WAVES * 64, [&](int j, int k) {
@@ -97,10 +103,12 @@
   const bt::rsrc_t adv_r = bt::make_rsrc(tr.adv, B32 * 4u), act_r = bt::make_rsrc(tr.action, B32);
   const uint32_t off_a = ((uint32_t)(2 * hf) * plane32 + (uint32_t)n) * 4u, off_b = off_a + plane32 * 4u;
   const uint32_t off_c = (4u * plane32 + (uint32_t)n) * 4u, off_s = (uint32_t)n * 4u, off_s1 = off_s + B32 * 4u;
+  const bt::rsrc_t mimg_r = bt::make_rsrc(mimg, (n_full + (tail != 0u ? 1u : 0u)) * bt::MIMG_TILE_BYTES);
   int since_flush = 0;
   struct TileOp {
     float xa, xb, xc, l0, l1, adv;
     int act;
+    bt::u32x4 m_lo, m_hi;
   };
   auto load_tile = [&](uint32_t g) {
     TileOp o;
@@ -117,6 +125,11 @@
     if (!JVP) {
       o.adv = bt::buf_f32(adv_r, off_s, soff);
       o.act = (int)bt::buf_u8(act_r, (uint32_t)n, g * 32u);
+    }
+    o.m_lo = o.m_hi = (bt::u32x4){0u, 0u, 0u, 0u};
+    if (CACHED) {
+      o.m_lo = bt::mimg_load(mimg_r, lane, g, 0);
+      o.m_hi = bt::mimg_load(mimg_r, lane, g, 1);
     }
     return o;
   };
@@ -152,18 +165,25 @@
       }
       return bt::layer1(fa, fw[t]);
     };
-    bt::f32x16 c = fwd(0);
-#pragma unroll
-    for (int t = 0; t < NT; ++t) {
-      bt::f32x16 cn = c;
-      if (t + 1 < NT) cn = fwd(t + 1);
-      if (!JVP) {
-#pragma unroll
-        for (int r = 0; r < 16; ++r) y0[r] = __builtin_fmaf(__builtin_fabsf(c[r]), w2d[t], y0[r]);
-      }
-      if (BWD) bt::mask_tile(c, ga[t]);
-      if (JVP) q = bt::masked_sum_tile(ga[t], idb, Fz, t, lane, q);
-      c = cn;
+    if (CACHED) {
+      bt::mimg_unpack(op_in.m_lo, op_in.m_hi, ga);
+#pragma unroll
+      for (int t = 0; t < NT; ++t) q = bt::masked_sum_tile(ga[t], idb, Fz, t, lane, q);
+    } else {
+      bt::f32x16 c = fwd(0);
+#pragma unroll
+      for (int t = 0; t < NT; ++t) {
+        bt::f32x16 cn = c;
+        if (t + 1 < NT) cn = fwd(t + 1);
+        if (!JVP) {
+#pragma unroll
+          for (int r = 0; r < 16; ++r) y0[r] = __builtin_fmaf(__builtin_fabsf(c[r]), w2d[t], y0[r]);
+        }
+        if (BWD) bt::mask_tile(c, ga[t]);
+        if (KEEP && (t & 1) != 0) bt::mimg_store_half(mimg_r, lane, g, t >> 1, ga);
+        if (JVP) q = bt::masked_sum_tile(ga[t], idb, Fz, t, lane, q);
+        c = cn;
+      }
     }
     float s0;
     if (JVP) {
@@ -252,7 +272,8 @@
       fold();
     }
   };
-  bt::walk_tiles<!JVP>(deal, n_full, tail, load_tile, tile);
+  if constexpr (CACHED) bt::walk_tiles_ahead<MIMG_AHEAD>(deal, n_full, tail, load_tile, tile);
+  else bt::walk_tiles<!JVP>(deal, n_full, tail, load_tile, tile);
   if (BWD && (since_flush != 0 || !flushed)) bt::flush(dm, acc64, IW, n, hf, !flushed);
   fold();
   const double r0 = bt::owner_sum(sum0, hf), r1 = bt::owner_sum(sum1, hf);
@@ -298,8 +319,21 @@
   }
 }
 
+static uint4 *mimg_for_write(rl_traj *t) {
+  const uint64_t tiles = (t->B + 31) / 32;
+  if (t->mimg_unavailable || tiles * bt::MIMG_TILE_BYTES >= (1ull << 31)) return nullptr;
+  try {
+    t->mem.ensure(t->mimg, tiles * bt::MIMG_TILE_UINT4);
+  } catch (const RlError &) {
+    (void)hipGetLastError();
+    t->mimg = nullptr;
+    t->mimg_unavailable = true;
+  }
+  return t->mimg;
+}
+
 bool launch_policy_v2(rl_traj *traj, const rl_mlp *policy, int mode, const float *d_tangent, uint64_t B_total,
-                      const int32_t *d_skip, float clip_lo, float clip_hi) {
+                      const int32_t *d_skip, float clip_lo, float clip_hi, bool keep_masks) {
   if (policy->general) return launch_gen_mfma(traj, policy, mode, d_tangent, B_total, d_skip, clip_lo, clip_hi);
   if (!fused_5_128_fits(traj, policy, 2)) return false;
   if (mode == PASS_DQN) return false;
@@ -312,18 +346,30 @@
   dim3 g(traj->nbV2), b(V2_WAVES * 64);
   hipStream_t s = traj->eng->stream;
   uint32_t P = (uint32_t)policy->P;
-  const TrajDev d = fused_traj_dev(traj, traj->guard_next_policy);
-#define BLAUNCH(MM)                                                                                                  \
-  hipLaunchKernelGGL((k_policy_bf16<MM, V2_WAVES>), g, b, 0, s, d, policy->d_params, wimg, d_tangent, traj->lp0,       \
-                     traj->slabA, traj->slabB, inv_B, P, d_skip, clip_lo, clip_hi, bt::SHARE_OLD, bt::SHARE_YOUNG)
-  if (mode == PASS_INIT) BLAUNCH(PASS_INIT);
-  else if (mode == PASS_JVP) BLAUNCH(PASS_JVP);
-  else if (mode == PASS_PPO) BLAUNCH(PASS_PPO);
+  const int form = traj->eng->fvp_form;
+  uint4 *mimg = nullptr;
+  if (mode == PASS_INIT) {
+    if (keep_masks && form != RL_FVP_RECOMPUTE) mimg = mimg_for_write(traj);
+    traj->mimg_epoch = mimg != nullptr ? traj->eng->call_epoch : 0;
+    traj->mimg_policy = policy;
+  } else if (mode == PASS_JVP && form != RL_FVP_RECOMPUTE && mimg_valid(traj, policy)) {
+    mimg = traj->mimg;
+  }
+  bool no_guard = false;
+  const TrajDev d = fused_traj_dev(traj, mode == PASS_JVP && mimg != nullptr ? no_guard : traj->guard_next_policy);
+#define BLAUNCH(...)                                                                                                 \
+  hipLaunchKernelGGL((k_policy_bf16<__VA_ARGS__>), g, b, 0, s, d, policy->d_params, wimg, d_tangent, traj->lp0,       \
+                     traj->slabA, traj->slabB, inv_B, P, d_skip, clip_lo, clip_hi, bt::SHARE_OLD, bt::SHARE_YOUNG, mimg)
+  if (mode == PASS_INIT && mimg != nullptr) BLAUNCH(PASS_INIT, V2_WAVES, false, true);
+  else if (mode == PASS_INIT) BLAUNCH(PASS_INIT, V2_WAVES);
+  else if (mode == PASS_JVP && mimg == nullptr) BLAUNCH(PASS_JVP, V2_WAVES);
+  else if (mode == PASS_JVP) BLAUNCH(PASS_JVP, V2_WAVES, false, true);
+  else if (mode == PASS_PPO) BLAUNCH(PASS_PPO, V2_WAVES);
   else {
     constexpr int EVAL_WAVES = 16;
     hipLaunchKernelGGL((k_policy_bf16<PASS_EVAL, EVAL_WAVES, true>), g, dim3(EVAL_WAVES * 64), 0, s, d,
                        policy->d_params, wimg, d_tangent, traj->lp0, traj->slabA, traj->slabB, inv_B, P, d_skip, clip_lo,
-                       clip_hi, 1u, 1u);
+                       clip_hi, 1u, 1u, mimg);
   }
 #undef BLAUNCH
   return true;
diff --git a/relearn_amd/csrc/kernels_update.hip b/relearn_amd/csrc/kernels_update.hip
--- a/relearn_amd/csrc/kernels_update.hip
+++ b/relearn_amd/csrc/kernels_update.hip
@@ -771,6 +771,7 @@
 }
 
 void launch_ls_set_params(rl_traj *traj, rl_mlp *policy, double ratio) {
+  traj->mimg_epoch = 0;
   ProfScope ps(traj->eng, RL_K_SMALL);
   hipLaunchKernelGGL(k_ls_set_params, dim3(1), dim3(SB), 0, traj->eng->stream, policy->d_params, traj->prev_params,
                      traj->descent, (uint32_t)policy->P, (float)ratio, traj->trpo, comm_err_word(traj->eng),
```

Measured after the change: 502.3 million env-steps/s (median of 6 runs). No clear change (+0.8%).
